# cchao0116/EasyDGL

Measured on AMD Instinct MI355X. Metric: sequences/sec (fwd+bwd+Adam) B=512 L=100 d=128 |I|=20K, higher is better.
Workload: dtype bf16

## Files before the change

### easydgl_amd/build.py

```python
from __future__ import annotations

import hashlib
import os
import subprocess
import sys
from concurrent.futures import ThreadPoolExecutor

HERE = os.path.dirname(os.path.abspath(__file__))
CSRC = os.path.join(HERE, "csrc")
OUT = os.path.join(HERE, "libeasydgl_hip.so")
SOURCES = ["k_misc.hip", "k_tpp.hip", "k_optim.hip", "k_adam_rows.hip", "k_reduce.hip", "k_data.hip", "k_encode.hip", "k_gemm.hip", "k_gemm2.hip", "k_layernorm.hip", "k_bimau_fwd.hip", "k_bimau_bwd.hip", "k_bimau_big.hip", "k_bimau_stream.hip",
           "k_score.hip", "k_ce.hip", "k_score_strip.hip", "k_score_stripw.hip", "k_eval_tile.hip", "k_eval_topk.hip", "k_eval_rank.hip", "k_eval_cand.hip", "k_cand_ce.hip", "k_shared_ce.hip", "k_sampled_loss.hip", "k_tattn.hip", "k_tiattn.hip", "k_timefn.hip", "k_coding.hip", "k_tail.hip", "k_segsum.hip", "k_gru.hip", "k_s2pnm.hip", "k_mate.hip", "k_tahe.hip"]
HEADERS = ["edgl_common.h", "lds_limit.h", "batch_prep.h", "tpp_math.h", "score_plan.h", "topk_select.h", "gemm_tile.h", "bimau_common.h", "bimau_fwd_impl.h", "bimau_bwd_impl.h", "red_batch.h", "tn_group.h", "encode_scatter.h", "strip_mma.h", "score_strip.h", "eval_sweep.h", "cand_gather.h", "sampled_dv.h", "tattn_common.h", os.path.join("..", "..", "include", "easydgl_hip.h")]
FLAGS = ["--offload-arch=gfx950", "-O3", "-std=c++17", "-fPIC", "-munsafe-fp-atomics", "-Wno-unused-result"]
EXTRA_FLAGS = {"k_bimau_fwd.hip": ["-mllvm", "-amdgpu-mfma-vgpr-form=1"],
               "k_bimau_bwd.hip": ["-mllvm", "-amdgpu-mfma-vgpr-form=1"],
               "k_bimau_big.hip": ["-mllvm", "-amdgpu-mfma-vgpr-form=1"],
               "k_bimau_stream.hip": ["-mllvm", "-amdgpu-mfma-vgpr-form=1"],
               "k_tattn.hip": ["-mllvm", "-amdgpu-mfma-vgpr-form=1"],
               "k_tiattn.hip": ["-mllvm", "-amdgpu-mfma-vgpr-form=1"],
               "k_timefn.hip": ["-mllvm", "-amdgpu-mfma-vgpr-form=1"],
               "k_score_strip.hip": ["-fno-slp-vectorize", "-Wno-unused-value"] + (["-DSTRIP_SAFE"] if os.environ.get("EDGL_STRIP_SAFE") else []),
               "k_score_stripw.hip": ["-fno-slp-vectorize", "-Wno-unused-value"] + (["-DSTRIP_SAFE"] if os.environ.get("EDGL_STRIP_SAFE") else [])}


def _hipcc() -> str:
    for c in (os.environ.get("HIPCC"), "/opt/rocm/bin/hipcc", "hipcc"):
        if c and (os.path.isabs(c) and os.path.exists(c) or not os.path.isabs(c)):
            return c
    raise RuntimeError("hipcc not found")


def _digest(paths, extra=()) -> str:
    h = hashlib.sha256()
    for e in extra:
        h.update(str(e).encode() + b"\0")
    for p in paths:
        with open(p, "rb") as f:
            h.update(os.path.basename(p).encode() + b"\0" + f.read() + b"\0")
    return h.hexdigest()


def _stamp_ok(target: str, digest: str) -> bool:
    stamp = target + ".sha256"
    return os.path.exists(target) and os.path.exists(stamp) and open(stamp).read().strip() == digest


def _write_stamp(target: str, digest: str) -> None:
    with open(target + ".sha256", "w") as f:
        f.write(digest + "\n")


def build(force: bool = False, verbose: bool = False) -> str:
    hipcc = _hipcc()
    objdir = os.path.join(CSRC, "obj")
    os.makedirs(objdir, exist_ok=True)
    hdrs = [os.path.join(CSRC, h) for h in HEADERS]
    jobs = []
    digests = {}
    for src in SOURCES:
        s = os.path.join(CSRC, src)
        o = os.path.join(objdir, src.replace(".hip", ".o"))
        digests[o] = _digest([s] + hdrs, FLAGS + EXTRA_FLAGS.get(src, []))
        if force or not _stamp_ok(o, digests[o]):
            jobs.append((s, o))

    def run(job):
        s, o = job
        cmd = [hipcc] + FLAGS + EXTRA_FLAGS.get(os.path.basename(s), []) + ["-c", s, "-o", o]
        r = subprocess.run(cmd, capture_output=True, text=True)
        if r.returncode != 0:
            raise RuntimeError("hipcc failed for %s:\n%s" % (s, r.stderr[-4000:]))
        _write_stamp(o, digests[o])
        if verbose:
            print("compiled", os.path.basename(s))
        return o

    if jobs:
        with ThreadPoolExecutor(max_workers=min(8, len(jobs))) as ex:
            list(ex.map(run, jobs))
    objs = [os.path.join(objdir, s.replace(".hip", ".o")) for s in SOURCES]
    link_digest = _digest([], [digests[o] for o in objs])
    if force or jobs or not _stamp_ok(OUT, link_digest):
        cmd = [hipcc, "--offload-arch=gfx950", "-shared", "-fPIC", "-o", OUT] + objs
        r = subprocess.run(cmd, capture_output=True, text=True)
        if r.returncode != 0:
            raise RuntimeError("link failed:\n" + r.stderr[-4000:])
        _write_stamp(OUT, link_digest)
    return OUT


if __name__ == "__main__":
    print(build(force="--force" in sys.argv, verbose=True))
```

### easydgl_amd/csrc/bimau_bwd_impl.h

```cpp
#pragma once
#include <algorithm>

#include "bimau_common.h"

#ifdef EDGL_PHASE_TIMING
extern __device__ unsigned long long g_phase_cycles[16];
#endif

namespace bimau {


constexpr int KY_ECH = 8;
constexpr int KY_NY = EP / KY_ECH;
constexpr int KY_BLOCKS = 384;

constexpr int WG_NJ64 = 4;
constexpr int big_nj(int dh) { return dh == 64 ? WG_NJ64 : 32 / (dh / 16); }
inline int big_row_splits(int dh, int E) {
    const int nc = big_nj(dh) * 16;
    const int groups = std::max(1, (dh * E + nc - 1) / nc);
    return std::max(16, 512 / groups);
}

struct WsLayout { size_t dz, dh, rowdot, dsc, wpart, total; };
inline WsLayout ws_layout(int B, int T_, int C, int H, int E, long dsc_rows = 0) {
    const int dh = C / H;
    const bool big = dh >= 64;
    const size_t R = (size_t)B * H * T_;
    WsLayout w;
    size_t o = 0;
    auto take = [&](size_t bytes) { const size_t at = o; o += (bytes + 255) & ~(size_t)255; return at; };
    w.dz = take(R * EP * sizeof(float));
    w.dh = take((size_t)(big ? 1 : KY_NY) * R * dh * sizeof(float));
    w.rowdot = take(R * sizeof(float));
    w.dsc = take((size_t)(dsc_rows > 0 ? dsc_rows : (long)B * H) * EP * sizeof(float));
    w.wpart = take((size_t)(big ? big_row_splits(dh, E) : KY_BLOCKS) * ((size_t)(dh + 3) * dh * E + EP) * sizeof(float));
    w.total = o;
    return w;
}

struct BwdP {
    const void* qkvt; const int64_t* ids; const float* spans; const uint8_t* marks; const char* pack;
    const void* d_out; const float* d_lam_ext; const float* lam; const float* z; const void* hin;
    int B, T, C, H, E;
    float rate; const uint64_t* rng; uint32_t stream_id;
    void* d_qkvt;
    float* dz_ws; float* dh_ws; float* rowdot_ws; float* dsc_part; float* wpart;
    int waves;
    int flags;
    int noskip;
    const uint32_t* dbits;
    float qk_scale;
    const void* tpp_desc; int tpp_M; const float* tpp_sums; float tpp_coef;
    const int32_t* order;
    float* tpp_part;
};

template <typename T>
__device__ __forceinline__ void st_frag(T* dst, const f32x4& a) {
    Frag4<T> f = frag_from_acc<T>(a);
    if constexpr (sizeof(T) == 4) *reinterpret_cast<uint4*>(dst) = *reinterpret_cast<uint4*>(&f);
    else *reinterpret_cast<uint2*>(dst) = *reinterpret_cast<uint2*>(&f);
}

template <typename T, int DT, int NT, int EC, bool PREF = true, int FL = -1, bool DB = false, bool TP = false, bool SK = false>
__global__ __launch_bounds__(256) void bimau_bwd_sweep1_kernel(BwdP p) {
    constexpr int dh = 16 * DT, Tp = 16 * NT, LDT = Tp + 4;
    extern __shared__ __attribute__((aligned(16))) char smem[];
    const int E = EC ? EC : p.E;
    const int lane = threadIdx.x & 63, wave = __builtin_amdgcn_readfirstlane(threadIdx.x >> 6);
    const long slot = (long)blockIdx.x * p.waves + wave;
    if (slot >= (long)p.B * p.H) return;
    const int sb = (int)(slot / p.H), head = (int)(slot % p.H);
    const int b = p.order ? __builtin_amdgcn_readfirstlane(p.order[sb]) : sb;
    const long job = (long)b * p.H + head;
    const long bp = (long)head * p.B + b;
    const int g4 = (lane >> 4) * 4, l15 = lane & 15;
    constexpr bool SWZ = img_swz<T>();
    const int g4s = SWZ ? swz_col<16>(l15, g4) : g4;
    int cw[DT];
#pragma unroll
    for (int ub = 0; ub < DT; ++ub) cw[ub] = SWZ ? swz_col<16 * DT>(l15, ub * 16 + g4) : ub * 16 + g4;

    constexpr bool TR = sizeof(T) == 2;
    constexpr size_t EXTRA = TR ? 0 : (size_t)EP * LDT;
    constexpr size_t MASK_ELEMS = (size_t)Tp * sizeof(float) / sizeof(T);
    constexpr size_t WAVE_ELEMS = 2 * (size_t)Tp * dh + (size_t)Tp * EP + EXTRA + MASK_ELEMS;
    T* Ks = reinterpret_cast<T*>(smem) + (size_t)wave * WAVE_ELEMS;
    T* Vs = Ks + Tp * dh;
    T* Ms = Vs + Tp * dh;
    T* MTs = Ms + Tp * EP;
    const T* qkvt = reinterpret_cast<const T*>(p.qkvt) + (long)b * p.T * 4 * p.C;
    const T* dout = reinterpret_cast<const T*>(p.d_out) + (long)b * p.T * p.C;
    T* dqkvt = reinterpret_cast<T*>(p.d_qkvt) + (long)b * p.T * 4 * p.C;
    const int ldq = 4 * p.C;
    const KeyMask<NT> km = stage_wave<T, DT, NT, EC>(
        qkvt + p.C + head * dh, Ks, nullptr, static_cast<const T*>(nullptr), static_cast<T*>(nullptr), static_cast<T*>(nullptr),
        qkvt + 2 * p.C + head * dh, Vs, nullptr, ldq, p.marks + (long)b * p.T * E, E, Ms, TR ? nullptr : MTs,
        p.ids + (long)b * p.T, reinterpret_cast<float*>(Ks + WAVE_ELEMS - MASK_ELEMS), p.T, LDT, lane);
    __builtin_amdgcn_fence(__ATOMIC_RELEASE, "wavefront");
    __builtin_amdgcn_wave_barrier();

    const PackDims pd = pack_dims<T>(dh, E);
    const float* iscs_g = reinterpret_cast<const float*>(p.pack + pd.off_f32) + 3 * pd.JE + EP;
    float isc[4];
#pragma unroll
    for (int i = 0; i < 4; ++i) isc[i] = iscs_g[g4 + i];

    const float cscale = p.qk_scale > 0.f ? p.qk_scale : rsqrtf((float)dh);
    const DropKey dk = make_dropkey(p.rng, p.stream_id, p.rate);
    const Frag4<T> ident = identity_frag<T>(lane);
    const f32x4 zero4 = {0.f, 0.f, 0.f, 0.f};

    struct QOps { Frag4<T> qf[DT], dof[DT]; float4 z; float lam[4], dlx[4]; uint32_t kb; uint32_t nmw; float spr; };
    const float* dlx_src = p.d_lam_ext ? p.d_lam_ext : p.lam;
    const float dlx_on = p.d_lam_ext ? 1.0f : 0.0f;
    TppDesc td{};
    int tp_novf = 0;
    float tp_k = 0.f;
    if constexpr (TP) {
        td = tpp_desc(p.tpp_desc, p.B, p.T, p.tpp_M);
        tp_novf = __builtin_amdgcn_readfirstlane(td.novf[b]);
        int cnt;
        if (p.tpp_sums) {
            cnt = reinterpret_cast<const int*>(p.tpp_sums)[4];
        } else {
            cnt = 0;
            for (int i = lane; i < p.B; i += 64) cnt += td.cntp[i];
            for (int o = 32; o > 0; o >>= 1) cnt += __shfl_xor(cnt, o, 64);
        }
        tp_k = -p.tpp_coef / ((float)cnt * (float)p.H);
        if (job == 0 && lane == 0) reinterpret_cast<int*>(p.tpp_part)[2 * p.B * p.H] = cnt;
    }
    auto load_q = [&](int qt) {
        QOps o;
        const int q = min(qt * 16 + l15, p.T - 1);
        const long row = bp * p.T + q;
#pragma unroll
        for (int ub = 0; ub < DT; ++ub) {
            o.qf[ub] = frag_ld<T>(qkvt + (long)q * ldq + head * dh + ub * 16 + g4);
            o.dof[ub] = frag_ld<T>(dout + (long)q * p.C + head * dh + ub * 16 + g4);
        }
        o.z = *reinterpret_cast<const float4*>(p.z + row * EP + g4);
        if constexpr (DB) o.kb = p.dbits[(bp * NT + qt) * 64 + lane];
        if constexpr (TP) {
            const float4 l4 = *reinterpret_cast<const float4*>(p.lam + row * EC + g4);
            o.lam[0] = l4.x; o.lam[1] = l4.y; o.lam[2] = l4.z; o.lam[3] = l4.w;
            o.dlx[0] = 0.f; o.dlx[1] = 0.f; o.dlx[2] = 0.f; o.dlx[3] = 0.f;
            o.nmw = td.nmw[((long)b * p.T + q) * 4 + (lane >> 4)];
            o.spr = td.spr[(long)b * p.T + q];
        } else if constexpr (EC == 16) {
            const float4 l4 = *reinterpret_cast<const float4*>(p.lam + row * EC + g4), d4 = *reinterpret_cast<const float4*>(dlx_src + row * EC + g4);
            o.lam[0] = l4.x; o.lam[1] = l4.y; o.lam[2] = l4.z; o.lam[3] = l4.w;
            o.dlx[0] = d4.x; o.dlx[1] = d4.y; o.dlx[2] = d4.z; o.dlx[3] = d4.w;
        } else {
#pragma unroll
            for (int i = 0; i < 4; ++i) {
                const int e = min(g4 + i, E - 1);
                o.lam[i] = p.lam[row * E + e];
                o.dlx[i] = dlx_src[row * E + e];
            }
        }
        return o;
    };
    auto mask_q = [&](QOps& o, bool ok) {
#pragma unroll
        for (int ub = 0; ub < DT; ++ub)
            if (!ok) o.dof[ub] = frag_zero<T>();
#pragma unroll
        for (int i = 0; i < 4; ++i) {
            const bool oke = ok && (EC == 16 || (g4 + i) < E);
            o.lam[i] = oke ? o.lam[i] : 0.f;
            o.dlx[i] = oke ? o.dlx[i] * dlx_on : 0.f;
        }
    };
    PH_DECL
    auto run = [&](auto nk_c) {
    constexpr int NK = decltype(nk_c)::value, K0 = NT - NK;
    const KeyMask<NK> kmk = keymask_tail<NK, NT>(km);
    float dsc_acc[4] = {0.f, 0.f, 0.f, 0.f}, tp_a = 0.f, tp_b = 0.f;
    f32x4 dVa[DT][NK];
#pragma unroll
    for (int u = 0; u < DT; ++u)
#pragma unroll
        for (int kt = 0; kt < NK; ++kt) dVa[u][kt] = zero4;
    QOps qcur = load_q(0);
    touch_regs(qcur);
    float pend_dz[4] = {0.f, 0.f, 0.f, 0.f}, pend_rowdot = 0.f;
    int pend_q = p.T;
    auto flush_pending = [&]() {
        if (pend_q < p.T) {
            *reinterpret_cast<float4*>(p.dz_ws + (bp * p.T + pend_q) * EP + g4) = make_float4(pend_dz[0], pend_dz[1], pend_dz[2], pend_dz[3]);
            if (lane < 16) p.rowdot_ws[bp * p.T + pend_q] = pend_rowdot;
        }
    };
    for (int qt = 0; qt < NT; ++qt) {
        asm volatile("" ::: "memory");
        const int q = qt * 16 + l15;
        const bool qok = q < p.T;
        QOps qnext;
        if constexpr (PREF) qnext = load_q(qt + 1 < NT ? qt + 1 : qt);
        asm volatile("" ::: "memory");
        mask_q(qcur, qok);
        if constexpr (TP) {
            float gr[4] = {0.f, 0.f, 0.f, 0.f};
            tpp_slot(qcur.lam, qcur.nmw, qcur.spr, qok && qcur.spr >= 0.f, tp_k, gr, tp_a, tp_b);
            for (int j = 0; j < tp_novf; ++j) {
                const int tj = td.ovf_pos[(long)b * td.M + j];
                if ((tj >> 4) != qt) continue;
                tpp_slot(qcur.lam, td.ovf_nm[((long)b * td.M + j) * 4 + (lane >> 4)], qcur.spr, qok && q == tj, tp_k, gr, tp_a, tp_b);
            }
#pragma unroll
            for (int i = 0; i < 4; ++i) qcur.dlx[i] = gr[i];
        }
        const float zq4[4] = {qcur.z.x, qcur.z.y, qcur.z.z, qcur.z.w};
        f32x4 s[NK];
#pragma unroll
        for (int kt = 0; kt < NK; ++kt) {
            f32x4 a = zero4;
#pragma unroll
            for (int ub = 0; ub < DT; ++ub)
                a = mma16(frag_ld<T>(Ks + ((K0 + kt) * 16 + l15) * dh + cw[ub]), qcur.qf[ub], a);
            s[kt] = a;
        }
// ... 415 lines not shown
```

### easydgl_amd/csrc/k_bimau_big.hip

```cpp
#include "bimau_bwd_impl.h"
#include "bimau_fwd_impl.h"
#include <type_traits>

namespace {
using namespace bimau;

struct IntP {
    const void* hin; const float* spans; const char* pack; const float* dz;
    long R; int B, T, E;
    float* z_out; float* lam;
    float* dh_out;
    float* wpart; const float* dsc_part; long njobs;
};

__device__ __forceinline__ void copy16(const char* src, char* dst, int bytes) {
    for (int i = threadIdx.x * 16; i < bytes; i += blockDim.x * 16)
        *reinterpret_cast<uint4*>(dst + i) = *reinterpret_cast<const uint4*>(src + i);
}

typedef unsigned int u32x4 __attribute__((ext_vector_type(4)));
typedef unsigned int u32x2 __attribute__((ext_vector_type(2)));
template <typename T, int DT, bool WITH_R>
struct MarkChunk {
    static constexpr int dh = 16 * DT, LDC = dh + 4;
// ... 306 lines not shown
        for (int r = 0; r < 4; ++r) {
            const int q = min(qt * 16 + g4 + r, p.T - 1);
            o.spn[r] = p.spans[(long)bb * p.T + q];
            o.dz0[r] = p.dz[(rowq + q) * EP + e_lo];
            o.dz1[r] = p.dz[(rowq + q) * EP + e_hi];
        }
        return o;
    };
    const long tstep = (long)gridDim.x * 4;
    long t = (long)blockIdx.x * 4 + wave;
    Pre cur = load_tile(t);
    for (; t < ntile; t += tstep) {
        const Pre nxt = load_tile(t + tstep);
        const long bpq = t / ntq; const int qt = (int)(t - bpq * ntq);
        const bool okA = qt * 16 + l15 < p.T;
        Frag4<T> hA[DT], hB[DT];
#pragma unroll
        for (int ub = 0; ub < DT; ++ub) {
            hA[ub] = okA ? cur.hA[ub] : frag_zero<T>();
            hB[ub] = frag_from_acc<T>(mma16(hA[ub], ident, zero4));
        }
        float spn[4];
        bool rok[4];
#pragma unroll
        for (int r = 0; r < 4; ++r) {
            rok[r] = qt * 16 + g4 + r < p.T;
            spn[r] = rok[r] ? cur.spn[r] : 0.f;
        }
#pragma unroll
        for (int jj = 0; jj < NJ; ++jj) {
            const bool hi_mark = (j0 + jj * 16) / dh > e_lo;
            f32x4 a = zero4;
#pragma unroll
            for (int ub = 0; ub < DT; ++ub) a = mma16(hA[ub], frag_ld<T>(Wc + (jj * 16 + l15) * LDW + ub * 16 + g4), a);
            const float ws = fc[jj * 16 + l15], bs = fc[NC + jj * 16 + l15], wv = fc[2 * NC + jj * 16 + l15];
            f32x4 du;
            float sdb = 0.f, sdws = 0.f, sdw = 0.f;
#pragma unroll
            for (int r = 0; r < 4; ++r) {
                const float dz = rok[r] ? (hi_mark ? cur.dz1[r] : cur.dz0[r]) : 0.f;
                const float z = sigmoid_pre(fmaf(spn[r], ws, a[r]) + bs);
                const float t2 = dz * z;
                du[r] = t2 * wv * (1.0f - z);
                sdb += du[r]; sdws += du[r] * spn[r]; sdw += t2;
            }
            adb[jj] += sdb; adws[jj] += sdws; adw[jj] += sdw;
            const Frag4<T> duf = frag_from_acc<T>(du);
#pragma unroll
            for (int ub = 0; ub < DT; ++ub) dW[jj][ub] = mma16(duf, hB[ub], dW[jj][ub]);
        }
        cur = nxt;
    }
    for (int w = 0; w < 4; ++w) {
        if (wave == w) {
#pragma unroll
            for (int jj = 0; jj < NJ; ++jj) {
                const float sb = group_sum4(adb[jj]), sws = group_sum4(adws[jj]), sw = group_sum4(adw[jj]);
                if (lane < 16) {
                    accs[dh * NC + jj * 16 + l15] += sws;
                    accs[(dh + 1) * NC + jj * 16 + l15] += sb;
                    accs[(dh + 2) * NC + jj * 16 + l15] += sw;
                }
#pragma unroll
                for (int ub = 0; ub < DT; ++ub)
#pragma unroll
                    for (int r = 0; r < 4; ++r) accs[(ub * 16 + l15) * NC + jj * 16 + g4 + r] += dW[jj][ub][r];
            }
        }
        __syncthreads();
    }
    float* dst = p.wpart + (long)blockIdx.x * NPARX;
    for (int i = threadIdx.x; i < (dh + 3) * NC; i += blockDim.x)
        if ((i % NC) < nval) dst[(long)(i / NC) * JE + j0 + (i % NC)] = accs[i];
    if (blockIdx.y == 0 && threadIdx.x < EP) {
        const long per = (p.njobs + gridDim.x - 1) / gridDim.x;
        const long a0 = blockIdx.x * per, a1 = min(p.njobs, a0 + per);
        float a = 0.f;
        for (long j = a0; j < a1; ++j) a += p.dsc_part[j * EP + threadIdx.x];
        dst[NPAR + threadIdx.x] = a;
    }
}

inline int row_blocks(long ntile, int tiles_per_wg) {
    return (int)std::max<long>(1, std::min<long>((ntile + tiles_per_wg - 1) / tiles_per_wg, 1024));
}

template <typename T, int DT>
int run_intensity_fwd(const FwdP& p, hipStream_t st) {
    constexpr int dh = 16 * DT;
    IntP ip{};
    ip.hin = p.hin_out; ip.spans = p.spans; ip.pack = p.pack; ip.R = (long)p.B * p.H * p.T; ip.B = p.B; ip.T = p.T; ip.E = p.E;
    ip.z_out = p.z_out; ip.lam = p.lam;
    const size_t smem = (size_t)MarkChunk<T, DT, false>::BYTES * (big_double_buffer<T, DT>() ? 2 : 1);
    auto k = intensity_fwd_big_kernel<T, DT>;
    EDGL_LDS_LIMIT(k, smem, "edgl_bimau_fwd");
    const long ntile = (long)p.B * p.H * ((p.T + 15) / 16);
    hipLaunchKernelGGL(k, dim3(row_blocks(ntile, 8)), dim3(256), smem, st, ip);
    EDGL_LAUNCH_CHECK();
    return EDGL_OK;
}

template <typename T, int DT, int NT>
int fwd_big(FwdP p, hipStream_t st) {
    int rc = launch_fwd_e<T, DT, NT, 0, 1>(p, st);
    if (rc) return rc;
    rc = run_intensity_fwd<T, DT>(p, st);
    if (rc) return rc;
    return launch_fwd_e<T, DT, NT, 0, 2>(p, st);
}

template <typename T, int DT>
int run_intensity_bwd_big(const BwdP& p, long dsc_rows, hipStream_t st) {
    constexpr int dh = 16 * DT;
    const long jobs = (long)p.B * p.H;
    const int JE = dh * p.E;
    const int RS = big_row_splits(dh, p.E);
    IntP ip{};
    ip.hin = p.hin; ip.spans = p.spans; ip.pack = p.pack; ip.dz = p.dz_ws; ip.R = (long)p.B * p.H * p.T; ip.B = p.B; ip.T = p.T;
    ip.E = p.E; ip.dh_out = p.dh_ws; ip.wpart = p.wpart; ip.dsc_part = p.dsc_part; ip.njobs = dsc_rows;
    const long ntile = jobs * ((p.T + 15) / 16);
    const size_t smem_r = (size_t)MarkChunk<T, DT, true>::BYTES * (big_double_buffer<T, DT>() ? 2 : 1);
    auto kr = intensity_bwd_rows_big_kernel<T, DT>;
    EDGL_LDS_LIMIT(kr, smem_r, "edgl_bimau_bwd");
    hipLaunchKernelGGL(kr, dim3(row_blocks(ntile, 8)), dim3(256), smem_r, st, ip);
    EDGL_LAUNCH_CHECK();
    constexpr int NC = WGroup<DT>::NJ * 16;
    const size_t smem_w = (size_t)NC * (dh + 4) * sizeof(T) + (size_t)(3 * NC + (dh + 3) * NC) * sizeof(float);
    auto kw = intensity_bwd_weights_big_kernel<T, DT>;
    EDGL_LDS_LIMIT(kw, smem_w, "edgl_bimau_bwd");
    hipLaunchKernelGGL(kw, dim3(RS, (JE + NC - 1) / NC), dim3(256), smem_w, st, ip);
    EDGL_LAUNCH_CHECK();
    return EDGL_OK;
}

template <typename T, int DT, int NT>
int bwd_big(BwdP p, char* ws, float* dW1, float* db1, float* dw, float* dscaling, hipStream_t st) {
    constexpr int dh = 16 * DT, Tp = 16 * NT, LDT = Tp + 4;
    constexpr bool TR = sizeof(T) == 2;
    const WsLayout wl = ws_layout(p.B, p.T, p.C, p.H, p.E);
    p.dz_ws = reinterpret_cast<float*>(ws + wl.dz); p.dh_ws = reinterpret_cast<float*>(ws + wl.dh);
    p.rowdot_ws = reinterpret_cast<float*>(ws + wl.rowdot);
    p.dsc_part = reinterpret_cast<float*>(ws + wl.dsc); p.wpart = reinterpret_cast<float*>(ws + wl.wpart);
    const long jobs = (long)p.B * p.H;
    edgl_prof_begin(EDGL_KERNEL_BIMAU_BWD_ALL, st);
    {
        const size_t wave_bytes = (2 * (size_t)Tp * dh + (size_t)Tp * EP + (TR ? 0 : (size_t)EP * LDT)) * sizeof(T) + (size_t)Tp * sizeof(float);
        int waves = 4;
        while (waves > 1 && waves * wave_bytes > 64 * 1024) waves >>= 1;
        const size_t smem = waves * wave_bytes;
        EDGL_REQUIRE(smem <= 160 * 1024, EDGL_ERR_SHAPE, "edgl_bimau_bwd: sweep 1 needs %zu B of LDS (dh=%d T=%d)", smem, dh, p.T);
        p.waves = waves;
        auto kern = bimau_bwd_sweep1_kernel<T, DT, NT, 0, false>;
        EDGL_LDS_LIMIT(kern, smem, "edgl_bimau_bwd");
        hipLaunchKernelGGL(kern, dim3((unsigned)((jobs + waves - 1) / waves)), dim3(64 * waves), smem, st, p);
        EDGL_LAUNCH_CHECK();
    }
    {
        const int rc = run_intensity_bwd_big<T, DT>(p, jobs, st);
        if (rc) return rc;
    }
    {
        const size_t wave_bytes = (3 * (size_t)Tp * dh + (size_t)Tp * EP + (TR ? 0 : (size_t)dh * LDT)) * sizeof(T) + (size_t)Tp * sizeof(float);
        int waves = 4;
        while (waves > 1 && waves * wave_bytes > 80 * 1024) waves >>= 1;
        const size_t smem = waves * wave_bytes;
        EDGL_REQUIRE(smem <= 160 * 1024, EDGL_ERR_SHAPE, "edgl_bimau_bwd: sweep 2 needs %zu B of LDS (dh=%d T=%d)", smem, dh, p.T);
        p.waves = waves;
        edgl_prof_begin(EDGL_KERNEL_BIMAU_BWD, st);
        if constexpr (DT * NT > 32) {
            auto k0 = bimau_bwd_sweep2_kernel<T, DT, NT, 0, 1, false, -1, false, 2, 0>;
            auto k1 = bimau_bwd_sweep2_kernel<T, DT, NT, 0, 1, false, -1, false, 2, 1>;
            EDGL_LDS_LIMIT(k0, smem, "edgl_bimau_bwd");
            EDGL_LDS_LIMIT(k1, smem, "edgl_bimau_bwd");
            hipLaunchKernelGGL(k0, dim3((unsigned)((jobs + waves - 1) / waves)), dim3(64 * waves), smem, st, p);
            hipLaunchKernelGGL(k1, dim3((unsigned)((jobs + waves - 1) / waves)), dim3(64 * waves), smem, st, p);
        } else {
            auto kern = bimau_bwd_sweep2_kernel<T, DT, NT, 0, 1, false>;
            EDGL_LDS_LIMIT(kern, smem, "edgl_bimau_bwd");
            hipLaunchKernelGGL(kern, dim3((unsigned)((jobs + waves - 1) / waves)), dim3(64 * waves), smem, st, p);
        }
        edgl_prof_end(EDGL_KERNEL_BIMAU_BWD, st);
        edgl_prof_end(EDGL_KERNEL_BIMAU_BWD_ALL, st);
        EDGL_LAUNCH_CHECK();
    }
    return reduce_wparts(p.wpart, big_row_splits(dh, p.E), dh, p.E, dW1, db1, dw, dscaling, st);
}

constexpr bool big_ok(size_t esize, int DT, int NT) { return esize == 2 ? NT <= 8 : (DT == 4 ? NT <= 7 : NT <= 4); }
template <typename T, int DT, int NT>
int fwd_big_or_error(const FwdP& p, hipStream_t st) {
    if constexpr (big_ok(sizeof(T), DT, NT)) return fwd_big<T, DT, NT>(p, st);
    edgl_set_error("edgl_bimau_fwd: head dim %d with T=%d in f32 not supported (f32: dh 64: T <= 112, dh 128: T <= 64; bf16: T <= 128)", 16 * DT, p.T);
    return EDGL_ERR_SHAPE;
}
template <typename T>
int fwd_dispatch(const FwdP& p, hipStream_t st) {
    const int dh = p.C / p.H, nt = (p.T + 15) / 16;
#define EDGL_BIG_CASES(DT_)                                                                                              \
    switch (nt) {                                                                                                        \
        case 1: return fwd_big_or_error<T, DT_, 1>(p, st); case 2: return fwd_big_or_error<T, DT_, 2>(p, st);            \
        case 3: return fwd_big_or_error<T, DT_, 3>(p, st); case 4: return fwd_big_or_error<T, DT_, 4>(p, st);            \
        case 5: return fwd_big_or_error<T, DT_, 5>(p, st); case 6: return fwd_big_or_error<T, DT_, 6>(p, st);            \
        case 7: return fwd_big_or_error<T, DT_, 7>(p, st); case 8: return fwd_big_or_error<T, DT_, 8>(p, st);            \
    }
    if (dh == 64) { EDGL_BIG_CASES(4) } else if (dh == 128) { EDGL_BIG_CASES(8) }
#undef EDGL_BIG_CASES
    edgl_set_error("edgl_bimau_fwd: head dim %d with T=%d not supported (head dims 64 / 128: T <= 128)", dh, p.T);
    return EDGL_ERR_SHAPE;
}
template <typename T, int DT, int NT>
int bwd_big_or_error(const BwdP& p, char* ws, float* dW1, float* db1, float* dw, float* dsc, hipStream_t st) {
    if constexpr (big_ok(sizeof(T), DT, NT)) return bwd_big<T, DT, NT>(p, ws, dW1, db1, dw, dsc, st);
    edgl_set_error("edgl_bimau_bwd: head dim %d with T=%d in f32 not supported (f32: dh 64: T <= 112, dh 128: T <= 64; bf16: T <= 128)", 16 * DT, p.T);
    return EDGL_ERR_SHAPE;
}
template <typename T>
int bwd_dispatch(const BwdP& p, char* ws, float* dW1, float* db1, float* dw, float* dsc, hipStream_t st) {
    const int dh = p.C / p.H, nt = (p.T + 15) / 16;
#define EDGL_BIG_CASES(DT_)                                                                                                            \
    switch (nt) {                                                                                                                      \
        case 1: return bwd_big_or_error<T, DT_, 1>(p, ws, dW1, db1, dw, dsc, st); case 2: return bwd_big_or_error<T, DT_, 2>(p, ws, dW1, db1, dw, dsc, st); \
        case 3: return bwd_big_or_error<T, DT_, 3>(p, ws, dW1, db1, dw, dsc, st); case 4: return bwd_big_or_error<T, DT_, 4>(p, ws, dW1, db1, dw, dsc, st); \
        case 5: return bwd_big_or_error<T, DT_, 5>(p, ws, dW1, db1, dw, dsc, st); case 6: return bwd_big_or_error<T, DT_, 6>(p, ws, dW1, db1, dw, dsc, st); \
        case 7: return bwd_big_or_error<T, DT_, 7>(p, ws, dW1, db1, dw, dsc, st); case 8: return bwd_big_or_error<T, DT_, 8>(p, ws, dW1, db1, dw, dsc, st); \
    }
    if (dh == 64) { EDGL_BIG_CASES(4) } else if (dh == 128) { EDGL_BIG_CASES(8) }
#undef EDGL_BIG_CASES
    edgl_set_error("edgl_bimau_bwd: head dim %d with T=%d not supported (head dims 64 / 128: T <= 128)", dh, p.T);
    return EDGL_ERR_SHAPE;
}

}

namespace bimau {
int big_fwd(const FwdP& p, int dtype, hipStream_t st) {
    if (!p.hin_out || !p.z_out) {
        edgl_set_error("edgl_bimau_fwd: head dims >= 64 run as three launches and need `saved` (edgl_bimau_saved_bytes) as scratch, also for inference");
        return EDGL_ERR_WORKSPACE;
    }
    return dtype == EDGL_F32 ? fwd_dispatch<float>(p, st) : fwd_dispatch<bf16>(p, st);
}
int big_bwd(const BwdP& p, char* ws, float* dW1, float* db1, float* dw, float* dsc, int dtype, hipStream_t st) {
    return dtype == EDGL_F32 ? bwd_dispatch<float>(p, ws, dW1, db1, dw, dsc, st) : bwd_dispatch<bf16>(p, ws, dW1, db1, dw, dsc, st);
}
int intensity_fwd_rows(const FwdP& p, int dtype, hipStream_t st) {
    const bool f = dtype == EDGL_F32;
    switch (p.C / p.H) {
        case 16: return f ? run_intensity_fwd<float, 1>(p, st) : run_intensity_fwd<bf16, 1>(p, st);
        case 32: return f ? run_intensity_fwd<float, 2>(p, st) : run_intensity_fwd<bf16, 2>(p, st);
        case 64: return f ? run_intensity_fwd<float, 4>(p, st) : run_intensity_fwd<bf16, 4>(p, st);
        case 128: return f ? run_intensity_fwd<float, 8>(p, st) : run_intensity_fwd<bf16, 8>(p, st);
    }
    edgl_set_error("edgl_bimau_fwd: head dim %d not supported (16, 32, 64 or 128)", p.C / p.H);
    return EDGL_ERR_SHAPE;
}
int intensity_bwd_big(const BwdP& p, long dsc_rows, float* dW1, float* db1, float* dw, float* dsc, int dtype, hipStream_t st) {
    const bool f = dtype == EDGL_F32;
    const int dh = p.C / p.H;
    int rc;
    if (dh == 64) rc = f ? run_intensity_bwd_big<float, 4>(p, dsc_rows, st) : run_intensity_bwd_big<bf16, 4>(p, dsc_rows, st);
    else if (dh == 128) rc = f ? run_intensity_bwd_big<float, 8>(p, dsc_rows, st) : run_intensity_bwd_big<bf16, 8>(p, dsc_rows, st);
    else { edgl_set_error("edgl_bimau_bwd: head dim %d has no streamed-weights intensity backward (64 or 128)", dh); return EDGL_ERR_SHAPE; }
    if (rc) return rc;
    return reduce_wparts(p.wpart, big_row_splits(dh, p.E), dh, p.E, dW1, db1, dw, dsc, st);
}
}
```

### easydgl_amd/csrc/k_bimau_bwd.hip

```cpp
#include <algorithm>
#include <cstdlib>

#include "bimau_bwd_impl.h"

#ifdef EDGL_PHASE_TIMING
__device__ unsigned long long g_phase_cycles[16];
#endif

namespace {
using namespace bimau;

template <typename T>
constexpr int intensity_bwd_nreg(int DT) {
    return KY_ECH * DT * DT * 4 + (sizeof(T) == 2 ? (KY_ECH / 4) * DT * 4 : 2 * KY_ECH * DT) + KY_ECH * DT;
}

struct MlpP {
    const void* hin; const float* dz_ws; const float* spans; const char* pack;
    long R; int B, T, E; float* dh_ws; float* wpart; const float* dsc_part; long njobs;
    int slab_epi;
};

template <typename T, int DT, int EC>
__global__ __launch_bounds__(256, (sizeof(T) == 2 && DT == 1) ? 3 : 1) void intensity_bwd_kernel(MlpP p) {
// ... 194 lines not shown
                    slab[(RX + (ee * DT + d) * 2 + 1) * 64] = adws[ee][d];
                }
                slab[(RW + ee * DT + d) * 64] = adw[ee][d];
            }
        __syncthreads();
        const float* sl = reinterpret_cast<const float*>(smem);
        auto sum4 = [&](int reg, int ln) {
            const float* q = sl + reg * 64 + ln;
            return (q[0] + q[NREG * 64]) + (q[2 * NREG * 64] + q[3 * NREG * 64]);
        };
        for (int i = threadIdx.x; i < NPAR; i += blockDim.x) {
            const int row = i / JE, j = i - row * JE;
            const int jt = j >> 4, jl = j & 15, e = jt / DT, d = jt - e * DT, ee = e - e0;
            if (ee < 0 || ee >= ECH) continue;
            float v;
            if (row < dh) {
                v = sum4((((ee * DT + d) * DT + (row >> 4)) * 4) + (jl & 3), (jl >> 2) * 16 + (row & 15));
            } else if (row == dh + 2) {
                const int reg = RW + ee * DT + d;
                v = (sum4(reg, jl) + sum4(reg, 16 + jl)) + (sum4(reg, 32 + jl) + sum4(reg, 48 + jl));
            } else if constexpr (MX) {
                const int reg = RX + ((ee / 4) * DT + d) * 4 + (jl & 3), ln = (jl >> 2) * 16 + 3 * (ee % 4);
                v = row == dh + 1 ? sum4(reg, ln) : sum4(reg, ln + 1) + sum4(reg, ln + 2);
            } else {
                const int reg = RX + (ee * DT + d) * 2 + (row == dh ? 1 : 0);
                v = (sum4(reg, jl) + sum4(reg, 16 + jl)) + (sum4(reg, 32 + jl) + sum4(reg, 48 + jl));
            }
            p.wpart[(long)blockIdx.x * NPARX + i] = v;
        }
    } else {
    for (int w = 0; w < 4; ++w) {
        if (wave == w) {
#pragma unroll
            for (int ee = 0; ee < ECH; ++ee) {
                const int e = e0 + ee;
                if (EC == 16 || e < E) {
#pragma unroll
                    for (int d = 0; d < DT; ++d) {
                        const int jt = e * DT + d;
                        const float sw = group_sum4(adw[ee][d]);
                        if (lane < 16) accs[WROW + 2 * JE + jt * 16 + l15] += sw;
                        if constexpr (MX) {
                            const int c0 = 3 * (ee % 4);
#pragma unroll
                            for (int r = 0; r < 4; ++r) {
                                const float x = dWx[ee / 4][d][r];
                                const float nb = __int_as_float(__builtin_amdgcn_update_dpp(0, __float_as_int(x), 0x101, 0xf, 0xf, true));
                                const int j = jt * 16 + g4 + r;
                                if (l15 == c0 || l15 == c0 + 1) accs[l15 == c0 ? WROW + JE + j : WROW + j] += l15 == c0 ? x : x + nb;
                            }
                        } else {
                            const float sb = group_sum4(adb[ee][d]), sws = group_sum4(adws[ee][d]);
                            if (lane < 16) {
                                const int j = jt * 16 + l15;
                                accs[WROW + j] += sws;
                                accs[WROW + JE + j] += sb;
                            }
                        }
#pragma unroll
                        for (int ub = 0; ub < DT; ++ub)
#pragma unroll
                            for (int r = 0; r < 4; ++r) {
                                const int j = jt * 16 + g4 + r, u = ub * 16 + l15;
                                accs[j * (dh + 1) + u] += dW[ee][d][ub][r];
                            }
                    }
                }
            }
        }
        __syncthreads();
    }
    for (int i = threadIdx.x; i < NPAR; i += blockDim.x) {
        const int e = (i % JE) / dh;
        const int row = i / JE, j = i - row * JE;
        if (e >= e0 && e < e0 + ECH) p.wpart[(long)blockIdx.x * NPARX + i] = row < dh ? accs[j * (dh + 1) + row] : accs[WROW + (row - dh) * JE + j];
    }
    }
    if (blockIdx.y == 0) {
        const long per = (p.njobs + gridDim.x - 1) / gridDim.x;
        const long j0 = blockIdx.x * per, j1 = min(p.njobs, j0 + per);
        const int e = threadIdx.x & 15, sl = threadIdx.x >> 4;
        float a = 0.f;
        for (long j = j0 + sl; j < j1; j += 16) a += p.dsc_part[j * EP + e];
        __syncthreads();
        accs[sl * EP + e] = a;
        __syncthreads();
        if (threadIdx.x < EP) {
            float v = 0.f;
#pragma unroll
            for (int k = 0; k < 16; ++k) v += accs[k * EP + threadIdx.x];
            p.wpart[(long)blockIdx.x * NPARX + NPAR + threadIdx.x] = v;
        }
    }
    PH_MARK(7);
    PH_FLUSH(0);
}

template <typename T>
size_t intensity_bwd_lds(int dh, int E) {
    const int NACC = dh * E * (dh + 4);
    return pack_dims<T>(dh, E).bytes + ((size_t)((NACC + 3) & ~3) + 4 * (16 * KY_ECH + 16)) * sizeof(float);
}

template <typename T, int DT>
int launch_intensity_bwd(const BwdP& p, long dsc_rows, hipStream_t st) {
    constexpr int dh = 16 * DT;
    MlpP mp{p.hin, p.dz_ws, p.spans, p.pack, (long)p.B * p.H * p.T, p.B, p.T, p.E, p.dh_ws, p.wpart, p.dsc_part, dsc_rows, 0};
    size_t smem_b = intensity_bwd_lds<T>(dh, p.E);
    const size_t slab_b = (size_t)4 * intensity_bwd_nreg<T>(DT) * 64 * sizeof(float);
    mp.slab_epi = slab_b <= std::max(smem_b, (size_t)52 * 1024);
    if (mp.slab_epi) smem_b = std::max(smem_b, slab_b);
    EDGL_REQUIRE(smem_b <= 160 * 1024, EDGL_ERR_SHAPE, "edgl_bimau_bwd: intensity kernel needs %zu B of LDS", smem_b);
    EDGL_REQUIRE((long)p.B * p.H * p.T < (1l << 31) - 16, EDGL_ERR_SHAPE, "edgl_bimau_bwd: B*H*T = %ld rows exceed the 32-bit row index", (long)p.B * p.H * p.T);
    auto kb = intensity_bwd_kernel<T, DT, 0>;
    EDGL_LDS_LIMIT(kb, smem_b, "edgl_bimau_bwd");
    hipLaunchKernelGGL(kb, dim3(KY_BLOCKS, KY_NY), dim3(256), smem_b, st, mp);
    EDGL_LAUNCH_CHECK();
    return EDGL_OK;
}

template <typename T, int DT, int NT>
int launch_bwd(BwdP p, char* ws, float* dW1, float* db1, float* dw, float* dscaling, hipStream_t st) {
    constexpr int dh = 16 * DT, Tp = 16 * NT, LDT = Tp + 4;
    const PackDims pd = pack_dims<T>(dh, p.E);
    const WsLayout wl = ws_layout(p.B, p.T, p.C, p.H, p.E);
    p.dz_ws = reinterpret_cast<float*>(ws + wl.dz); p.dh_ws = reinterpret_cast<float*>(ws + wl.dh);
    p.rowdot_ws = reinterpret_cast<float*>(ws + wl.rowdot);
    p.dsc_part = reinterpret_cast<float*>(ws + wl.dsc); p.wpart = reinterpret_cast<float*>(ws + wl.wpart);
    const long jobs = (long)p.B * p.H;
    constexpr bool TR = sizeof(T) == 2;
    edgl_prof_begin(EDGL_KERNEL_BIMAU_BWD_ALL, st);
    {
        const size_t wave_bytes = (2 * (size_t)Tp * dh + (size_t)Tp * EP + (TR ? 0 : (size_t)EP * LDT)) * sizeof(T) + (size_t)Tp * sizeof(float);
        int waves = 4;
        while (waves > 1 && waves * wave_bytes > 64 * 1024) waves >>= 1;
        const size_t smem = waves * wave_bytes;
        p.waves = waves;
        constexpr bool SPEC = sizeof(T) == 2 && DT == 1;
        auto kern = p.E == 16 ? bimau_bwd_sweep1_kernel<T, DT, NT, 16> : bimau_bwd_sweep1_kernel<T, DT, NT, 0>;
        if constexpr (SPEC) {
            if (p.flags == 0) kern = p.E == 16 ? bimau_bwd_sweep1_kernel<T, DT, NT, 16, true, 0> : bimau_bwd_sweep1_kernel<T, DT, NT, 0, true, 0>;
            if constexpr (NT <= 8) {
                constexpr bool SKC = NT >= 2;
                const bool sk = SKC && p.flags == 0 && p.E == 16 && bimau_skip_enabled() && !p.noskip;
                const bool db = p.dbits && p.rate > 0.f;
                if (p.flags == 0 && p.E == 16 && db) kern = sk ? bimau_bwd_sweep1_kernel<T, DT, NT, 16, true, 0, true, false, SKC> : bimau_bwd_sweep1_kernel<T, DT, NT, 16, true, 0, true>;
                else if (sk) kern = bimau_bwd_sweep1_kernel<T, DT, NT, 16, true, 0, false, false, SKC>;
                if (p.tpp_desc) {
                    if (sk) kern = db ? bimau_bwd_sweep1_kernel<T, DT, NT, 16, true, 0, true, true, SKC> : bimau_bwd_sweep1_kernel<T, DT, NT, 16, true, 0, false, true, SKC>;
                    else kern = db ? bimau_bwd_sweep1_kernel<T, DT, NT, 16, true, 0, true, true> : bimau_bwd_sweep1_kernel<T, DT, NT, 16, true, 0, false, true>;
                }
            }
        }
        EDGL_LDS_LIMIT(kern, smem, "edgl_bimau_bwd");
        hipLaunchKernelGGL(kern, dim3((unsigned)((jobs + waves - 1) / waves)), dim3(64 * waves), smem, st, p);
        EDGL_LAUNCH_CHECK();
    }
    {
        const int rc = launch_intensity_bwd<T, DT>(p, jobs, st);
        if (rc) return rc;
    }
    {
        const size_t wave_bytes = (3 * (size_t)Tp * dh + (size_t)Tp * EP + (TR ? 0 : (size_t)dh * LDT)) * sizeof(T) + (size_t)Tp * sizeof(float);
        int waves = 4;
        while (waves > 1 && waves * wave_bytes > 80 * 1024) waves >>= 1;
        const size_t smem = waves * wave_bytes;
        EDGL_REQUIRE(smem <= 160 * 1024, EDGL_ERR_SHAPE, "edgl_bimau_bwd: needs %zu B of LDS", smem);
        p.waves = waves;
        constexpr bool SPEC = sizeof(T) == 2 && DT == 1;
        auto kern = p.E == 16 ? bimau_bwd_sweep2_kernel<T, DT, NT, 16> : bimau_bwd_sweep2_kernel<T, DT, NT, 0>;
        if constexpr (SPEC) {
            if (p.flags == 0) kern = p.E == 16 ? bimau_bwd_sweep2_kernel<T, DT, NT, 16, KY_NY, true, 0> : bimau_bwd_sweep2_kernel<T, DT, NT, 0, KY_NY, true, 0>;
            if constexpr (NT <= 8) {
                constexpr bool SKC = NT >= 2;
                const bool sk = SKC && p.flags == 0 && p.E == 16 && bimau_skip_enabled() && !p.noskip;
                if (p.flags == 0 && p.E == 16 && p.dbits && p.rate > 0.f) kern = sk ? bimau_bwd_sweep2_kernel<T, DT, NT, 16, KY_NY, true, 0, true, 1, 0, SKC> : bimau_bwd_sweep2_kernel<T, DT, NT, 16, KY_NY, true, 0, true>;
                else if (sk) kern = bimau_bwd_sweep2_kernel<T, DT, NT, 16, KY_NY, true, 0, false, 1, 0, SKC>;
            }
        }
        EDGL_LDS_LIMIT(kern, smem, "edgl_bimau_bwd");
        edgl_prof_begin(EDGL_KERNEL_BIMAU_BWD, st);
        hipLaunchKernelGGL(kern, dim3((unsigned)((jobs + waves - 1) / waves)), dim3(64 * waves), smem, st, p);
        edgl_prof_end(EDGL_KERNEL_BIMAU_BWD, st);
        edgl_prof_end(EDGL_KERNEL_BIMAU_BWD_ALL, st);
        EDGL_LAUNCH_CHECK();
    }
    return reduce_wparts(p.wpart, KY_BLOCKS, dh, p.E, dW1, db1, dw, dscaling, st);
}

template <typename T, int DT>
int dispatch_nt(BwdP p, char* ws, float* dW1, float* db1, float* dw, float* dsc, hipStream_t st) {
    switch ((p.T + 15) / 16) {
        case 1: return launch_bwd<T, DT, 1>(p, ws, dW1, db1, dw, dsc, st);
        case 2: return launch_bwd<T, DT, 2>(p, ws, dW1, db1, dw, dsc, st);
        case 3: return launch_bwd<T, DT, 3>(p, ws, dW1, db1, dw, dsc, st);
        case 4: return launch_bwd<T, DT, 4>(p, ws, dW1, db1, dw, dsc, st);
        case 5: return launch_bwd<T, DT, 5>(p, ws, dW1, db1, dw, dsc, st);
        case 6: return launch_bwd<T, DT, 6>(p, ws, dW1, db1, dw, dsc, st);
        case 7: return launch_bwd<T, DT, 7>(p, ws, dW1, db1, dw, dsc, st);
        case 8: return launch_bwd<T, DT, 8>(p, ws, dW1, db1, dw, dsc, st);
        case 9: return launch_bwd<T, DT, 9>(p, ws, dW1, db1, dw, dsc, st);
        case 10: return launch_bwd<T, DT, 10>(p, ws, dW1, db1, dw, dsc, st);
        case 11: return launch_bwd<T, DT, 11>(p, ws, dW1, db1, dw, dsc, st);
        case 12: return launch_bwd<T, DT, 12>(p, ws, dW1, db1, dw, dsc, st);
        case 13: return launch_bwd<T, DT, 13>(p, ws, dW1, db1, dw, dsc, st);
    }
    edgl_set_error("edgl_bimau_bwd: T=%d not supported (T <= 208)", p.T);
    return EDGL_ERR_SHAPE;
}

}

namespace bimau {
int intensity_bwd_small(const BwdP& p, long dsc_rows, float* dW1, float* db1, float* dw, float* dsc, int dtype, hipStream_t st) {
    const bool f = dtype == EDGL_F32;
    const int dh = p.C / p.H;
    int rc;
    if (dh == 16) rc = f ? launch_intensity_bwd<float, 1>(p, dsc_rows, st) : launch_intensity_bwd<bf16, 1>(p, dsc_rows, st);
    else if (dh == 32) rc = f ? launch_intensity_bwd<float, 2>(p, dsc_rows, st) : launch_intensity_bwd<bf16, 2>(p, dsc_rows, st);
    else { edgl_set_error("edgl_bimau_bwd: head dim %d has no weights-in-LDS intensity backward (16 or 32)", dh); return EDGL_ERR_SHAPE; }
    if (rc) return rc;
    return reduce_wparts(p.wpart, KY_BLOCKS, dh, p.E, dW1, db1, dw, dsc, st);
}
}

extern "C" long edgl_bimau_bwd_workspace_ex(int B, int T, int C, int H, int E, int dtype, int flags) {
    if (H <= 0 || C % H) return -1;
    const int form = bimau::bimau_form(T, C, H, dtype == EDGL_BF16 ? EDGL_BF16 : EDGL_F32, flags);
    return (long)ws_layout_form(B, T, C, H, E, form).total;
}
extern "C" long edgl_bimau_bwd_workspace(int B, int T, int C, int H, int E, int dtype) {
    return edgl_bimau_bwd_workspace_ex(B, T, C, H, E, dtype, 0);
}

extern "C" int edgl_bimau_mark_group(int C, int H, int dtype) {
    if (H <= 0 || C % H || (dtype != EDGL_F32 && dtype != EDGL_BF16)) return -1;
    const int dh = C / H;
    if (dh >= 64) return bimau::EP;
    for (int E = bimau::EP; E >= 1; --E) {
        const size_t b = dtype == EDGL_BF16 ? intensity_bwd_lds<bf16>(dh, E) : intensity_bwd_lds<float>(dh, E);
        if (b <= 160 * 1024) return E;
    }
    return -1;
}

extern "C" int edgl_bimau_bwd_db(const void* qkvt, const int64_t* ids, const float* spans, const uint8_t* marks,
                                 const void* pack, const void* d_out, const float* d_lam_ext, const float* lam,
                                 const void* saved, int B, int T, int C, int H, int E, float drop_rate,
                                 const uint64_t* rng_state, uint32_t stream_id, const uint32_t* dropbits, float qk_scale, void* d_qkvt,
                                 float* dW1, float* db1, float* dw, float* dscaling, void* workspace, int flags, int dtype, void* stream);
extern "C" int edgl_bimau_bwd(const void* qkvt, const int64_t* ids, const float* spans, const uint8_t* marks,
                              const void* pack, const void* d_out, const float* d_lam_ext, const float* lam,
                              const void* saved, int B, int T, int C, int H, int E, float drop_rate,
                              const uint64_t* rng_state, uint32_t stream_id, void* d_qkvt, float* dW1, float* db1,
                              float* dw, float* dscaling, void* workspace, int flags, int dtype, void* stream) {
    return edgl_bimau_bwd_db(qkvt, ids, spans, marks, pack, d_out, d_lam_ext, lam, saved, B, T, C, H, E, drop_rate, rng_state, stream_id,
                             nullptr, 0.f, d_qkvt, dW1, db1, dw, dscaling, workspace, flags, dtype, stream);
}
static int bimau_bwd_impl(const void* qkvt, const int64_t* ids, const float* spans, const uint8_t* marks,
                          const void* pack, const void* d_out, const float* d_lam_ext, const float* lam,
                          const void* saved, int B, int T, int C, int H, int E, float drop_rate,
                          const uint64_t* rng_state, uint32_t stream_id, const uint32_t* dropbits, float qk_scale, void* d_qkvt,
                          float* dW1, float* db1, float* dw, float* dscaling, void* workspace, const void* tpp_desc, int tpp_M,
                          const float* tpp_sums, float tpp_coef, float* tpp_part, const int32_t* order, int flags, int dtype, void* stream) {
    EDGL_REQUIRE(qkvt && ids && spans && marks && pack && d_out && lam && saved && d_qkvt && dW1 && db1 && dw && dscaling && workspace,
                 EDGL_ERR_NULL, "edgl_bimau_bwd: null pointer");
    EDGL_REQUIRE(B > 0 && T > 0 && H > 0 && C % H == 0 && E >= 1 && E <= bimau::EP, EDGL_ERR_SHAPE,
                 "edgl_bimau_bwd: bad shape B=%d T=%d C=%d H=%d E=%d", B, T, C, H, E);
    EDGL_REQUIRE(dtype == EDGL_F32 || dtype == EDGL_BF16, EDGL_ERR_DTYPE, "edgl_bimau_bwd: bad dtype %d", dtype);
    EDGL_REQUIRE(drop_rate == 0.f || rng_state, EDGL_ERR_NULL, "edgl_bimau_bwd: dropout without rng_state");
    EDGL_REQUIRE((double)B * H * T * T < 4294967296.0, EDGL_ERR_SHAPE, "edgl_bimau_bwd: H*B*T*T must be < 2^32");
    BwdP p{};
    p.qkvt = qkvt; p.ids = ids; p.spans = spans; p.marks = marks; p.pack = (const char*)pack; p.d_out = d_out;
    p.d_lam_ext = d_lam_ext; p.lam = lam;
    const bimau::SavedLayout sl = bimau::saved_layout(B, T, C, H, dtype == EDGL_BF16 ? 2 : 4);
    p.hin = (const char*)saved + sl.off_hin;
    p.z = reinterpret_cast<const float*>((const char*)saved + sl.off_z);
    p.B = B; p.T = T; p.C = C; p.H = H; p.E = E; p.rate = drop_rate; p.rng = rng_state;
    p.noskip = (flags & EDGL_MAU_NO_SKIP) ? 1 : 0; flags &= ~EDGL_MAU_NO_SKIP;
    p.stream_id = stream_id; p.d_qkvt = d_qkvt; p.flags = flags; p.dbits = dropbits; p.qk_scale = qk_scale;
    p.tpp_desc = tpp_desc; p.tpp_M = tpp_M; p.tpp_sums = tpp_sums; p.tpp_coef = tpp_coef; p.tpp_part = tpp_part; p.order = order;
    EDGL_REQUIRE(!tpp_desc || (dtype == EDGL_BF16 && C / H == 16 && E == 16 && T <= 128 && flags == 0 && tpp_part && tpp_M > 0 && !d_lam_ext),
                 EDGL_ERR_SHAPE, "edgl_bimau_bwd_tpp: the fused TPP form exists for bf16, head dim 16, 16 marks, T <= 128, BiMAU flags "
                 "(C/H=%d E=%d T=%d flags=%d)", C / H, E, T, flags);
    hipStream_t st = (hipStream_t)stream;
    const int dh = C / H;
    char* ws = (char*)workspace;
    const int form = bimau::bimau_form(T, C, H, dtype, flags);
    p.flags = flags & ~EDGL_MAU_STREAM;
    if (form < 0) {
        edgl_set_error("edgl_bimau_bwd: head dim %d with T=%d not supported (head dims 16, 32, 64 or 128; T <= %d)", dh, T, bimau::STREAM_MAX_T);
        return EDGL_ERR_SHAPE;
    }
    if (form == 1) {
        EDGL_REQUIRE(!tpp_desc, EDGL_ERR_SHAPE, "edgl_bimau_bwd_tpp: the fused TPP form does not exist on the key-streamed path (T=%d, T <= 128)", T);
        const WsLayout wl = ws_layout_form(B, T, C, H, E, 1);
        p.dz_ws = reinterpret_cast<float*>(ws + wl.dz); p.dh_ws = reinterpret_cast<float*>(ws + wl.dh);
        p.rowdot_ws = reinterpret_cast<float*>(ws + wl.rowdot);
        p.dsc_part = reinterpret_cast<float*>(ws + wl.dsc); p.wpart = reinterpret_cast<float*>(ws + wl.wpart);
        const bimau::SavedLayoutStream ss = bimau::saved_layout_stream(B, T, C, H, dtype == EDGL_BF16 ? 2 : 4);
        return bimau::stream_bwd(p, reinterpret_cast<const float*>((const char*)saved + ss.off_stats), dW1, db1, dw, dscaling, dtype, st);
    }
    if (dtype == EDGL_F32) {
        if (dh == 16) return dispatch_nt<float, 1>(p, ws, dW1, db1, dw, dscaling, st);
        if (dh == 32) return dispatch_nt<float, 2>(p, ws, dW1, db1, dw, dscaling, st);
    } else {
        if (dh == 16) return dispatch_nt<bf16, 1>(p, ws, dW1, db1, dw, dscaling, st);
        if (dh == 32) return dispatch_nt<bf16, 2>(p, ws, dW1, db1, dw, dscaling, st);
    }
// ... 45 lines not shown
```

### easydgl_amd/csrc/k_gemm2.hip

```cpp
#include <cstdlib>

#include "edgl_common.h"
#include <cstring>
#include "encode_scatter.h"
#include "tn_group.h"

typedef __attribute__((ext_vector_type(4))) short tr_s16x4;

namespace gemm2 {

__device__ __forceinline__ uint2 tr_read(const bf16* tile, int ld, int k0, int z0, int lane) {
    const int G = lane >> 4, s = lane & 15;
    const bf16* p = tile + (k0 + 4 * G + (s >> 2)) * ld + z0 + 4 * (s & 3);
    tr_s16x4 v = __builtin_amdgcn_ds_read_tr16_b64_v4i16((__attribute__((address_space(3))) tr_s16x4*)p);
    return *reinterpret_cast<uint2*>(&v);
}
__device__ __forceinline__ bf16x8 tr_frag32(const bf16* tile, int ld, int k0, int z0, int lane) {
    bf16x8 f;
    *reinterpret_cast<uint2*>(&f) = tr_read(tile, ld, k0, z0, lane);
    *(reinterpret_cast<uint2*>(&f) + 1) = tr_read(tile, ld, k0 + 16, z0, lane);
    return f;
}

struct EpiP {
    const float* bias; void* aux; int flags;
};

__device__ __forceinline__ int xcd_virtual_id(int b, int grid, int n_real) {
    if (grid & 7) return b < n_real ? b : -1;
    const int v = (b & 7) * (grid >> 3) + (b >> 3);
    return v < n_real ? v : -1;
}
static inline int xcd_grid(int n_real) { return (n_real + 7) / 8 * 8; }
__device__ __forceinline__ void epi_store4(const EpiP& e, bf16* C, void* Cany, long idx, int n, float x[4]) {
    if (e.flags & EDGL_EPI_BIAS) {
        const float4 b = *reinterpret_cast<const float4*>(e.bias + n);
        x[0] += b.x; x[1] += b.y; x[2] += b.z; x[3] += b.w;
    }
    if (e.flags & EDGL_EPI_SAVE_PRE) {
        Frag4<bf16> f = frag_from_acc<bf16>(f32x4{x[0], x[1], x[2], x[3]});
        *reinterpret_cast<uint2*>(reinterpret_cast<bf16*>(e.aux) + idx) = *reinterpret_cast<uint2*>(&f);
    }
    if (e.flags & EDGL_EPI_GELU) {
#pragma unroll
        for (int r = 0; r < 4; ++r) x[r] = gelu_t<bf16>(x[r]);
    }
    if (e.flags & EDGL_EPI_RELU) {
#pragma unroll
        for (int r = 0; r < 4; ++r) x[r] = fmaxf(x[r], 0.f);
    }
    if (e.flags & EDGL_EPI_MUL_DGELU) {
        const Frag4<bf16> a = frag_ld<bf16>(reinterpret_cast<const bf16*>(e.aux) + idx);
#pragma unroll
        for (int r = 0; r < 4; ++r) x[r] *= dgelu_t<bf16>(to_f32(a.v[r]));
    }
    if (e.flags & EDGL_EPI_OUT_F32) {
        float* c = reinterpret_cast<float*>(Cany) + idx;
        if (e.flags & EDGL_EPI_ACCUM) {
            const float4 o = *reinterpret_cast<const float4*>(c);
            x[0] += o.x; x[1] += o.y; x[2] += o.z; x[3] += o.w;
        }
        *reinterpret_cast<float4*>(c) = make_float4(x[0], x[1], x[2], x[3]);
    } else {
        if (e.flags & EDGL_EPI_ACCUM) {
            const Frag4<bf16> o = frag_ld<bf16>(C + idx);
#pragma unroll
            for (int r = 0; r < 4; ++r) x[r] += to_f32(o.v[r]);
        }
        Frag4<bf16> f = frag_from_acc<bf16>(f32x4{x[0], x[1], x[2], x[3]});
        *reinterpret_cast<uint2*>(C + idx) = *reinterpret_cast<uint2*>(&f);
    }
}

constexpr int S_NT = 256;
constexpr int S_ZB = 64;

struct StripP {
    const bf16* A; const bf16* B; void* C;
    int M, N, K, lda, ldb, ldc;
    EpiP epi;
};

struct StripEpi {
    bf16* Ostage; float* OstageF; const float* bias64;
    bool staged, fstage;
    uint4 pre_aux[2][2], pre_c[2][2];
};
__device__ __forceinline__ void strip_prefetch_combine(const StripP& p, StripEpi& e, int m0, int n0, int lane) {
    if (e.fstage) {
#pragma unroll
        for (int ix = 0; ix < 2; ++ix)
#pragma unroll
            for (int q = 0; q < 2; ++q) {
                const int m = min(m0 + ix * 16 + q * 8 + (lane >> 3), p.M - 1);
                const long idx = (long)m * p.ldc + n0 + (lane & 7) * 8;
                if (p.epi.flags & EDGL_EPI_MUL_DGELU) e.pre_aux[ix][q] = *reinterpret_cast<const uint4*>(reinterpret_cast<const bf16*>(p.epi.aux) + idx);
                if (p.epi.flags & EDGL_EPI_ACCUM) e.pre_c[ix][q] = *reinterpret_cast<const uint4*>(reinterpret_cast<const bf16*>(p.C) + idx);
            }
    }
}
__device__ __forceinline__ void strip_epilogue(const StripP& p, StripEpi& e, f32x4 (&acc)[4][2], int m0, int n0, int lane) {
    constexpr int LDO = 64 + 8, LDOF = 64 + 4;
    const int g4 = (lane >> 4) * 4, l15 = lane & 15;
    bf16* const Ostage = e.Ostage;
    float* const OstageF = e.OstageF;
    if (e.staged) {
#pragma unroll
        for (int ix = 0; ix < 2; ++ix) {
#pragma unroll
            for (int jz = 0; jz < 4; ++jz) {
                const int n = n0 + jz * 16 + g4;
                float x[4] = {acc[jz][ix][0], acc[jz][ix][1], acc[jz][ix][2], acc[jz][ix][3]};
                {
                    const float4 bb = *reinterpret_cast<const float4*>(e.bias64 + jz * 16 + g4);
                    x[0] += bb.x; x[1] += bb.y; x[2] += bb.z; x[3] += bb.w;
                }
                if (p.epi.flags & EDGL_EPI_SAVE_PRE) {
                    const int m = m0 + ix * 16 + l15;
                    if (m < p.M) {
                        Frag4<bf16> f = frag_from_acc<bf16>(f32x4{x[0], x[1], x[2], x[3]});
                        *reinterpret_cast<uint2*>(reinterpret_cast<bf16*>(p.epi.aux) + (long)m * p.ldc + n) = *reinterpret_cast<uint2*>(&f);
                    }
                }
                if (p.epi.flags & EDGL_EPI_GELU) {
#pragma unroll
                    for (int r = 0; r < 4; ++r) x[r] = gelu_t<bf16>(x[r]);
                }
                if (p.epi.flags & EDGL_EPI_RELU) {
#pragma unroll
                    for (int r = 0; r < 4; ++r) x[r] = fmaxf(x[r], 0.f);
                }
                Frag4<bf16> f = frag_from_acc<bf16>(f32x4{x[0], x[1], x[2], x[3]});
                *reinterpret_cast<uint2*>(Ostage + l15 * LDO + jz * 16 + g4) = *reinterpret_cast<uint2*>(&f);
            }
            __builtin_amdgcn_fence(__ATOMIC_RELEASE, "wavefront");
            __builtin_amdgcn_wave_barrier();
#pragma unroll
            for (int q = 0; q < 2; ++q) {
                const int lrow = q * 8 + (lane >> 3), cv = lane & 7, m = m0 + ix * 16 + lrow;
                const uint4 d = *reinterpret_cast<const uint4*>(Ostage + lrow * LDO + cv * 8);
                if (m < p.M) *reinterpret_cast<uint4*>(reinterpret_cast<bf16*>(p.C) + (long)m * p.ldc + n0 + cv * 8) = d;
            }
            __builtin_amdgcn_wave_barrier();
        }
    } else if (e.fstage) {
#pragma unroll
        for (int ix = 0; ix < 2; ++ix) {
#pragma unroll
            for (int jz = 0; jz < 4; ++jz) {
                const float4 bb = *reinterpret_cast<const float4*>(e.bias64 + jz * 16 + g4);
                *reinterpret_cast<float4*>(OstageF + l15 * LDOF + jz * 16 + g4) =
                    make_float4(acc[jz][ix][0] + bb.x, acc[jz][ix][1] + bb.y, acc[jz][ix][2] + bb.z, acc[jz][ix][3] + bb.w);
            }
            __builtin_amdgcn_fence(__ATOMIC_RELEASE, "wavefront");
            __builtin_amdgcn_wave_barrier();
#pragma unroll
            for (int q = 0; q < 2; ++q) {
                const int lrow = q * 8 + (lane >> 3), cv = lane & 7, m = m0 + ix * 16 + lrow;
                const float4 lo = *reinterpret_cast<const float4*>(OstageF + lrow * LDOF + cv * 8);
                const float4 hi = *reinterpret_cast<const float4*>(OstageF + lrow * LDOF + cv * 8 + 4);
                float x[8] = {lo.x, lo.y, lo.z, lo.w, hi.x, hi.y, hi.z, hi.w};
                if (p.epi.flags & EDGL_EPI_MUL_DGELU) {
                    const bf16x8 a = *reinterpret_cast<const bf16x8*>(&e.pre_aux[ix][q]);
#pragma unroll
                    for (int r = 0; r < 8; ++r) x[r] *= dgelu_t<bf16>(to_f32(a[r]));
                }
                if (p.epi.flags & EDGL_EPI_ACCUM) {
                    const bf16x8 o = *reinterpret_cast<const bf16x8*>(&e.pre_c[ix][q]);
#pragma unroll
                    for (int r = 0; r < 8; ++r) x[r] += to_f32(o[r]);
                }
                const Frag4<bf16> f0 = frag_from_acc<bf16>(f32x4{x[0], x[1], x[2], x[3]});
                const Frag4<bf16> f1 = frag_from_acc<bf16>(f32x4{x[4], x[5], x[6], x[7]});
                uint4 d;
                *reinterpret_cast<uint2*>(&d) = *reinterpret_cast<const uint2*>(&f0);
                *(reinterpret_cast<uint2*>(&d) + 1) = *reinterpret_cast<const uint2*>(&f1);
                if (m < p.M) *reinterpret_cast<uint4*>(reinterpret_cast<bf16*>(p.C) + (long)m * p.ldc + n0 + cv * 8) = d;
            }
            __builtin_amdgcn_wave_barrier();
        }
    } else {
#pragma unroll
        for (int ix = 0; ix < 2; ++ix) {
            const int m = m0 + ix * 16 + l15;
            if (m < p.M) {
#pragma unroll
// ... 294 lines not shown
        for (int i = 0; i < 4; ++i) {
            const int m = m0 + wm * 64 + i * 16 + l15;
#pragma unroll
            for (int j = 0; j < 4; ++j) {
                const int n = n0 + wn * 64 + j * 16 + g4;
                float x[4] = {acc[i][j][0], acc[i][j][1], acc[i][j][2], acc[i][j][3]};
                if (m < p.M) epi_store4(p.epi, reinterpret_cast<bf16*>(p.C), p.C, (long)m * p.ldc + n, n, x);
            }
        }
        return;
    }
    bf16* Os = reinterpret_cast<bf16*>(smem);
#pragma unroll
    for (int j = 0; j < 4; ++j) {
        const int nl = wn * 64 + j * 16 + g4;
        float4 b4 = make_float4(0.f, 0.f, 0.f, 0.f);
        if (p.epi.flags & EDGL_EPI_BIAS) b4 = *reinterpret_cast<const float4*>(p.epi.bias + n0 + nl);
#pragma unroll
        for (int i = 0; i < 4; ++i) {
            const int ml = wm * 64 + i * 16 + l15;
            const Frag4<bf16> f = frag_from_acc<bf16>(f32x4{acc[i][j][0] + b4.x, acc[i][j][1] + b4.y, acc[i][j][2] + b4.z, acc[i][j][3] + b4.w});
            *reinterpret_cast<uint2*>(Os + ml * G_LDO + nl) = *reinterpret_cast<const uint2*>(&f);
        }
    }
    lds_barrier();
    if constexpr (MAP) {
        dx_encode_epilogue(*x, Os, mb0, mt, vid % nbn, n0, p.ldc);
        return;
    }
    bf16* C = reinterpret_cast<bf16*>(p.C);
#pragma unroll
    for (int i = 0; i < 8; ++i) {
        const int v = tid + i * G_NT, r = v >> 4, cpc = (v & 15) * 8;
        if (m0 + r < p.M) *reinterpret_cast<uint4*>(C + (long)(m0 + r) * p.ldc + n0 + cpc) = *reinterpret_cast<const uint4*>(Os + r * G_LDO + cpc);
    }
#undef G_AROW
#undef G_LOAD_ONE
#undef G_LOAD
#undef G_STORE_ONE
#undef G_STORE
}

template <bool B_KC, bool EPI = false>
__global__ __launch_bounds__(G_NT, EPI ? 2 : 3) void tile_nn_kernel(StripP p) {
    extern __shared__ __attribute__((aligned(16))) char smem[];
    const int vid = xcd_virtual_id((int)blockIdx.x, (int)gridDim.x, ((p.M + G_BM - 1) / G_BM) * (p.N / G_BN));
    if (vid < 0) return;
    tile_nn_tile<B_KC, EPI, false>(p, vid, smem, nullptr);
}

constexpr int DXE_LDS = G_BM * G_LDO * (int)sizeof(bf16) + 4 * enc_scatter::SROWS * 4;
__device__ __forceinline__ void dx_encode_epilogue(const DxEncP& x, bf16* Os, int mb0, int mt, int jn, int n0, int ldc) {
    using namespace enc_scatter;
    static_assert(G_LDO == 128 + 8 && G_BM == SROWS, "the output tile is the scatter's row image");
    constexpr int C = 128;
    const EncBwdP& e = x.e;
    int* s_id = reinterpret_cast<int*>(Os + G_BM * G_LDO);
    int* s_lead = s_id + SROWS;
    float* s_nm = reinterpret_cast<float*>(s_lead + SROWS);
    const int tid = threadIdx.x, T = x.mapT, B = x.mapB;
    if (x.dx0_out) {
#pragma unroll
        for (int i = 0; i < 8; ++i) {
            const int v = tid + i * G_NT, r = v >> 4, cpc = (v & 15) * 8;
            if (mb0 + r < B) *reinterpret_cast<uint4*>(x.dx0_out + ((long)(mb0 + r) * T + mt) * ldc + n0 + cpc) = *reinterpret_cast<const uint4*>(Os + r * G_LDO + cpc);
        }
        lds_barrier();
    }
    const int rl = tid >> 5, c0 = (tid & 31) * 4;
    const DropKey dk = make_dropkey(e.rng, e.stream_id, e.rate);
    if (jn == 0) {
        if (tid < SROWS) s_id[tid] = mb0 + tid < B ? (int)e.ids[(long)(mb0 + tid) * T + mt] : 0;
        const bool adds = e.add1 != nullptr;
        Frag4<bf16> ga[16], gb[16];
        if (adds) {
#pragma unroll
            for (int k = 0; k < 16; ++k) {
                const long row = (long)min(mb0 + rl + 8 * k, B - 1) * T + mt;
                ga[k] = frag_ld<bf16>(reinterpret_cast<const bf16*>(e.add1) + row * C + c0);
                gb[k] = frag_ld<bf16>(reinterpret_cast<const bf16*>(e.add2) + row * C + c0);
            }
        }
        lds_barrier();
        if (tid < SROWS) {
            const int lead = scatter_leader(s_id, tid);
            s_lead[tid] = s_id[tid] == 0 ? -1 : lead;
        }
#pragma unroll
        for (int k = 0; k < 16; ++k) {
            const int r = rl + 8 * k;
            const long row = (long)(mb0 + r) * T + mt;
            Frag4<bf16> v;
            *reinterpret_cast<uint2*>(&v) = *reinterpret_cast<const uint2*>(Os + r * G_LDO + c0);
            if (adds) {
#pragma unroll
                for (int j = 0; j < 4; ++j) v.v[j] = from_f32<bf16>(to_f32(v.v[j]) + to_f32(ga[k].v[j]) + to_f32(gb[k].v[j]));
            }
            if (dk.thresh != 0u) {
                const uint32_t keep = drop_keep4(dk, (uint64_t)row * 3 * C + c0);
#pragma unroll
                for (int j = 0; j < 4; ++j)
                    if (!((keep >> j) & 1u)) v.v[j] = from_f32<bf16>(0.f);
            }
            *reinterpret_cast<uint2*>(Os + r * G_LDO + c0) = *reinterpret_cast<const uint2*>(&v);
        }
        lds_barrier();
        scatter_onehot_sum<8>(Os, s_id, s_lead, e.d_item, C, 0, e.sq * dk.scale);
        return;
    }
    if (jn == 2) {
        if (mb0 == 0 && mt == 0 && e.d_mark_zero)
            for (int i = tid; i < e.E * C; i += G_NT) e.d_mark_zero[i] = 0.f;
        if (tid < SROWS) {
            int nm = 0;
            if (mb0 + tid < B) {
                const uint8_t* mrow = e.marks + ((long)(mb0 + tid) * T + mt) * e.E;
                for (int q = 0; q < e.E; ++q) nm += mrow[q];
            }
            s_nm[tid] = (float)nm;
        }
        lds_barrier();
    }
    double a[4] = {0., 0., 0., 0.};
#pragma unroll
    for (int k = 0; k < 16; ++k) {
        const int r = rl + 8 * k;
        if (mb0 + r < B) {
            const long row = (long)(mb0 + r) * T + mt;
            Frag4<bf16> g;
            *reinterpret_cast<uint2*>(&g) = *reinterpret_cast<const uint2*>(Os + r * G_LDO + c0);
            float v[4];
#pragma unroll
            for (int j = 0; j < 4; ++j) v[j] = to_f32(g.v[j]);
            drop_apply4(dk, (uint64_t)row * 3 * C + jn * C + c0, v);
            const double w = jn == 2 ? (double)s_nm[r] : 1.;
#pragma unroll
            for (int j = 0; j < 4; ++j) a[j] += w * (double)v[j];
        }
    }
    lds_barrier();
    double* sm = reinterpret_cast<double*>(Os);
    *reinterpret_cast<double2*>(sm + rl * C + c0) = make_double2(a[0], a[1]);
    *reinterpret_cast<double2*>(sm + rl * C + c0 + 2) = make_double2(a[2], a[3]);
    lds_barrier();
    if (tid < C) {
        double s = 0.;
#pragma unroll
        for (int i = 0; i < 8; ++i) s += sm[i * C + tid];
        float* part = jn == 1 ? e.part_pos : e.part_mk;
        part[((long)(mb0 / G_BM) * T + mt) * C + tid] = (float)s;
    }
}

template <int TM>
__device__ __forceinline__ void tn_body(const TnP& p, int bx, int by, int bz, bf16* Xs, bf16* Ys);

__global__ __launch_bounds__(G_NT, 3) void dx_encode_kernel(StripP p, DxEncP x, RedBatch rb, TnGroupP g, int tn_blocks) {
    static_assert(sizeof(StripP) + sizeof(DxEncP) + sizeof(RedBatch) + sizeof(TnGroupP) + sizeof(int) < 4096, "kernel arguments: 4 KB");
    static_assert(T_NT == G_NT && 2 * T_BR * T_LD * (int)sizeof(bf16) <= DXE_LDS, "the TN tiles run in this kernel's workgroup shape and LDS");
    extern __shared__ __attribute__((aligned(16))) char smem[];
    const int bid0 = (int)blockIdx.x;
    const int bid = bid0 - tn_blocks;
    if (bid0 < tn_blocks) {
        const int vid = xcd_virtual_id(bid0, tn_blocks, g.blk0[g.n]);
        if (vid < 0) return;
        int j = 0;
        for (int i = 1; i < g.n; ++i)
            if (vid >= g.blk0[i]) j = i;
        const int local = vid - g.blk0[j];
        const int tn = g.tiles_n[j], tk = g.tiles_k[j];
        bf16* Xs = reinterpret_cast<bf16*>(smem);
        tn_body<128>(g.job[j], local % tn, (local / tn) % tk, local / (tn * tk), Xs, Xs + T_BR * T_LD);
        return;
    }
    if (bid >= x.gemm_blocks) {
        const int e = bid - x.gemm_blocks;
        bf16* Gs = reinterpret_cast<bf16*>(smem);
        int* s_id = reinterpret_cast<int*>(Gs + G_BM * G_LDO);
        if (e < x.lab_blocks)
            enc_scatter::scatter_block<8>(x.e, x.e.lab_blk0 + e, 0, Gs, s_id, s_id + 128, reinterpret_cast<float*>(s_id + 256), reinterpret_cast<float*>(s_id + 384));
        else
            reduce_rows_vec_block(rb, e - x.lab_blocks, reinterpret_cast<float4(*)[9]>(smem));
        return;
    }
    const int vid = xcd_virtual_id(bid, x.gemm_blocks, (x.mapB + G_BM - 1) / G_BM * x.mapT * (p.N / G_BN));
    if (vid < 0) return;
    tile_nn_tile<true, false, true>(p, vid, smem, &x);
}

template <bool B_KC, bool EPI = false>
static int launch_tile_nn(const StripP& p, hipStream_t st) {
    constexpr size_t a_el = (size_t)G_BM * G_LDK, b_el = B_KC ? (size_t)G_BN * G_LDK : (size_t)G_BK * G_LDN;
    const size_t smem = std::max((EPI ? 2 : 1) * (a_el + b_el) * sizeof(bf16), (size_t)G_BM * G_LDO * sizeof(bf16));
    auto k = tile_nn_kernel<B_KC, EPI>;
    EDGL_LDS_LIMIT(k, smem, "edgl_gemm (tile)");
    const int nbm = (p.M + G_BM - 1) / G_BM, nbn = p.N / G_BN;
    hipLaunchKernelGGL(k, dim3((unsigned)xcd_grid(nbm * nbn)), dim3(G_NT), smem, st, p);
    EDGL_LAUNCH_CHECK();
    return 1;
}

template <int TM>
__device__ __forceinline__ void tn_body(const TnP& p, int bx, int by, int bz, bf16* Xs, bf16* Ys) {
    constexpr int NI = TM / 32, LDT = TM + 16, PCS = TM / 8, NLD = T_BR * PCS / T_NT;
    const int tid = threadIdx.x, lane = tid & 63, wave = tid >> 6, wm = wave >> 1, wn = wave & 1;
    const int g4 = (lane >> 4) * 4, l15 = lane & 15;
    const int kf0 = by * TM, n0 = bx * TM;
    const int r_lo = bz * p.rows_per_split, r_hi = min(p.R, r_lo + p.rows_per_split);
    f32x4 acc[NI][NI];
#pragma unroll
    for (int i = 0; i < NI; ++i)
#pragma unroll
        for (int j = 0; j < NI; ++j) acc[i][j] = f32x4{0.f, 0.f, 0.f, 0.f};
    constexpr int NCS = NI / 2;
    f32x4 acc_cs[NCS];
#pragma unroll
    for (int j = 0; j < NCS; ++j) acc_cs[j] = f32x4{0.f, 0.f, 0.f, 0.f};
    const bool do_cs = p.with_colsum && by == 0;
    bf16x8 ones;
#pragma unroll
    for (int i = 0; i < 8; ++i) ones[i] = (__bf16)1.0f;
    uint4 px[NLD], py[NLD];
    int r0_cur = 0;
    auto load = [&](int r0) {
        r0_cur = r0;
#pragma unroll
        for (int i = 0; i < NLD; ++i) {
            const int v = tid + i * T_NT, row = v / PCS, cv = v % PCS, gr = min(r0 + row, r_hi - 1);
            const int cx = min(kf0 + cv * 8, p.Kf - 8), cy = min(n0 + cv * 8, p.N - 8);
            px[i] = *reinterpret_cast<const uint4*>(p.X + (long)gr * p.ldx + cx);
            py[i] = *reinterpret_cast<const uint4*>(p.Y + (long)gr * p.ldy + cy);
        }
    };
    auto store = [&]() {
#pragma unroll
        for (int i = 0; i < NLD; ++i) {
            const int v = tid + i * T_NT, row = v / PCS, cv = v % PCS;
            const bool ok = r0_cur + row < r_hi;
            *reinterpret_cast<uint4*>(Xs + row * LDT + cv * 8) = ok ? px[i] : make_uint4(0, 0, 0, 0);
            *reinterpret_cast<uint4*>(Ys + row * LDT + cv * 8) = ok ? py[i] : make_uint4(0, 0, 0, 0);
        }
    };
    const int nstep = (r_hi - r_lo + T_BR - 1) / T_BR;
    if (nstep > 0) { load(r_lo); store(); }
    __syncthreads();
    for (int st = 0; st < nstep; ++st) {
        const bool more = st + 1 < nstep;
        if (more) load(r_lo + (st + 1) * T_BR);
#pragma unroll
        for (int rb = 0; rb < T_BR / 32; ++rb) {
            bf16x8 af[NI], bf_[NI];
#pragma unroll
            for (int i = 0; i < NI; ++i) af[i] = tr_frag32(Xs, LDT, rb * 32, wm * (TM / 2) + i * 16, lane);
#pragma unroll
            for (int j = 0; j < NI; ++j) bf_[j] = tr_frag32(Ys, LDT, rb * 32, wn * (TM / 2) + j * 16, lane);
#pragma unroll
            for (int i = 0; i < NI; ++i)
#pragma unroll
                for (int j = 0; j < NI; ++j) acc[i][j] = __builtin_amdgcn_mfma_f32_16x16x32_bf16(af[i], bf_[j], acc[i][j], 0, 0, 0);
            if (do_cs) {
                if (wm) {
#pragma unroll
                    for (int j = 0; j < NCS; ++j) acc_cs[j] = __builtin_amdgcn_mfma_f32_16x16x32_bf16(ones, bf_[NCS + j], acc_cs[j], 0, 0, 0);
                } else {
#pragma unroll
                    for (int j = 0; j < NCS; ++j) acc_cs[j] = __builtin_amdgcn_mfma_f32_16x16x32_bf16(ones, bf_[j], acc_cs[j], 0, 0, 0);
                }
            }
        }
        lds_barrier();
        if (more) store();
        lds_barrier();
    }
    float* out = p.partial + (long)bz * (p.Kf + 1) * p.N;
#pragma unroll
    for (int i = 0; i < NI; ++i)
#pragma unroll
        for (int r = 0; r < 4; ++r) {
            const int kf = kf0 + wm * (TM / 2) + i * 16 + g4 + r;
            if (kf < p.Kf) {
#pragma unroll
                for (int j = 0; j < NI; ++j) {
                    const int n = n0 + wn * (TM / 2) + j * 16 + l15;
                    if (n < p.N) out[(long)kf * p.N + n] = acc[i][j][r];
                }
            }
        }
    if (do_cs && lane < 16) {
#pragma unroll
        for (int j = 0; j < NCS; ++j) {
            const int n = n0 + wn * (TM / 2) + (wm * NCS + j) * 16 + lane;
            if (n < p.N) out[(long)p.Kf * p.N + n] = acc_cs[j][0];
        }
    }
}

template <int TM>
__global__ __launch_bounds__(T_NT) void tn_gemm_kernel(TnP p) {
    extern __shared__ __attribute__((aligned(16))) char tn_smem[];
    bf16* Xs = reinterpret_cast<bf16*>(tn_smem);
    bf16* Ys = Xs + T_BR * (TM + 16);
    const int vid = xcd_virtual_id((int)blockIdx.x, (int)gridDim.x, p.nblocks);
    if (vid < 0) return;
    tn_body<TM>(p, vid % p.tiles_n, (vid / p.tiles_n) % p.tiles_k, vid / (p.tiles_n * p.tiles_k), Xs, Ys);
}

__global__ __launch_bounds__(T_NT) void tn_gemm_group_kernel(TnGroupP g) {
    extern __shared__ __attribute__((aligned(16))) char tn_smem[];
    bf16* Xs = reinterpret_cast<bf16*>(tn_smem);
    bf16* Ys = Xs + T_BR * (128 + 16);
    const int vid = xcd_virtual_id((int)blockIdx.x, (int)gridDim.x, g.blk0[g.n]);
    if (vid < 0) return;
    int j = 0;
    for (int i = 1; i < g.n; ++i)
        if (vid >= g.blk0[i]) j = i;
    const int local = vid - g.blk0[j];
    const int tn = g.tiles_n[j], tk = g.tiles_k[j];
    tn_body<128>(g.job[j], local % tn, (local / tn) % tk, local / (tn * tk), Xs, Ys);
}

}

using namespace gemm2;

template <int NKB, bool B_KC>
static int launch_stream(const StripP& p, hipStream_t st) {
    constexpr int K = 32 * NKB;
    constexpr size_t cel = B_KC ? (size_t)64 * (K + 16) : (size_t)K * (64 + 16);
    const bool fstage = (p.epi.flags & (EDGL_EPI_ACCUM | EDGL_EPI_MUL_DGELU)) && !(p.epi.flags & EDGL_EPI_OUT_F32);
    const size_t smem = 2 * cel * sizeof(bf16) + (size_t)((p.N + 3) / 4 * 4) * sizeof(float) +
                        (fstage ? (size_t)8 * 16 * (64 + 4) * sizeof(float) : (size_t)8 * 16 * (64 + 8) * sizeof(bf16));
    if (smem > 160 * 1024) return 0;
    auto k = strip_stream_kernel<NKB, B_KC>;
    EDGL_LDS_LIMIT(k, smem, "edgl_gemm (stream)");
    hipLaunchKernelGGL(k, dim3((p.M + 255) / 256), dim3(W_NT), smem, st, p);
    EDGL_LAUNCH_CHECK();
    return 1;
}

template <int NKB, bool B_KC>
static int launch_strip(const StripP& p, hipStream_t st) {
    constexpr int K = 32 * NKB;
    constexpr size_t wel = B_KC ? (size_t)128 * (K + 16) : (size_t)K * (128 + 16);
    const bool fstage = (p.epi.flags & (EDGL_EPI_ACCUM | EDGL_EPI_MUL_DGELU)) && !(p.epi.flags & EDGL_EPI_OUT_F32);
    const size_t smem = wel * sizeof(bf16) + 128 * sizeof(float) +
                        (fstage ? (size_t)8 * 16 * (64 + 4) * sizeof(float) : (size_t)8 * 16 * (64 + 8) * sizeof(bf16));
    if (smem > 160 * 1024) return 0;
    auto k = strip_gemm_kernel<NKB, B_KC>;
    EDGL_LDS_LIMIT(k, smem, "edgl_gemm (strip)");
    const int nparts = (p.N + 127) / 128;
    const int per_cu = std::max(1, (int)((160 * 1024) / smem));
    const int nstrip8 = (p.M + 255) / 256;
    const int gx = std::max(1, std::min(nstrip8, (256 * std::min(per_cu, 2)) / nparts));
    hipLaunchKernelGGL(k, dim3(gx, nparts), dim3(W_NT), smem, st, p);
    EDGL_LAUNCH_CHECK();
    return 1;
}

int edgl_gemm2_try_strip(const void* A, const void* B, void* C, int M, int N, int K, int lda, int ldb, int ldc, int b_kc,
                         const float* bias, void* aux, int flags, hipStream_t st) {
    const bool ok = (K % 32 == 0) && K >= 32 && (N % 64 == 0) && (lda % 8 == 0) && (ldb % 8 == 0) &&
                    (ldc % 4 == 0) && (((uintptr_t)A | (uintptr_t)B | (uintptr_t)C) & 15) == 0 &&
                    (!aux || ((uintptr_t)aux & 7) == 0) && (!bias || ((uintptr_t)bias & 15) == 0);
    if (!ok) return 0;
    StripP p{(const bf16*)A, (const bf16*)B, C, M, N, K, lda, ldb, ldc, EpiP{bias, aux, flags}};
    int rc;
    if (M >= 4096 && N >= 256 && (N % G_BN) == 0 && (K % G_BK) == 0 && K >= 128 && (flags & ~EDGL_EPI_BIAS) == 0 &&
        (ldc % 8) == 0)
        return b_kc ? launch_tile_nn<true>(p, st) : launch_tile_nn<false>(p, st);
    if (K > 512) {
        if (M >= 1024 && (N % G_BN) == 0 && (K % G_BK) == 0)
            return b_kc ? launch_tile_nn<true, true>(p, st) : launch_tile_nn<false, true>(p, st);
        return 0;
    }
    if (N >= 384 && (K == 384 || K == 512) && M >= 4096) {
        rc = 0;
        if (K == 384) rc = b_kc ? launch_stream<12, true>(p, st) : launch_stream<12, false>(p, st);
        else rc = b_kc ? launch_stream<16, true>(p, st) : launch_stream<16, false>(p, st);
        if (rc) return rc;
    }
#define STRIP_CASE(NKB)                                                             \
    case NKB: rc = b_kc ? launch_strip<NKB, true>(p, st) : launch_strip<NKB, false>(p, st); break;
    switch (K / 32) {
        STRIP_CASE(1) STRIP_CASE(2) STRIP_CASE(4) STRIP_CASE(8) STRIP_CASE(12) STRIP_CASE(16)
        default: rc = 0;
    }
#undef STRIP_CASE
    if (rc == 0 && M >= 1024 && (N % G_BN) == 0 && (K % G_BK) == 0 && K >= 128)
        return b_kc ? launch_tile_nn<true, true>(p, st) : launch_tile_nn<false, true>(p, st);
    return rc;
}

static int tn_cus() {
    static const int cus = [] {
        int dev = 0, n = 0;
        if (hipGetDevice(&dev) != hipSuccess || hipDeviceGetAttribute(&n, hipDeviceAttributeMultiprocessorCount, dev) != hipSuccess || n <= 0) n = 256;
        return n;
    }();
    return cus;
}
static int tn_choose_splits(int R, int tiles, double flop, double out_elems, int cap) { return tn_choose_splits_on(tn_cus(), R, tiles, flop, out_elems, cap); }
static int tn_splits(int R, int Kf, int N) {
    const int tiles = ((Kf + 127) / 128) * ((N + 127) / 128);
    return tn_choose_splits(R, tiles, 2.0 * R * Kf * N, (double)(Kf + 1) * N, 1 << 20);
}
long edgl_gemm2_tn_workspace(int R, int Kf, int N) { return (long)tn_splits(R, Kf, N) * (Kf + 1) * N; }

static int tn_reduce(const float* workspace, int splits, float* C, int Kf, int N, float* dbias, int accumulate, hipStream_t st) {
    if (dbias && dbias == C + (long)Kf * N)
        return edgl_reduce_rows(workspace, splits, (Kf + 1) * N, (long)(Kf + 1) * N, C, accumulate, st);
    int rc = edgl_reduce_rows(workspace, splits, Kf * N, (long)(Kf + 1) * N, C, accumulate, st);
    if (rc) return rc;
    if (dbias) rc = edgl_reduce_rows(workspace + (long)Kf * N, splits, N, (long)(Kf + 1) * N, dbias, accumulate, st);
    return rc;
}

thread_local bool g_tn_defer = false;
thread_local int g_tn_n = 0;
thread_local TnQueued g_tn_q[TN_MAX_JOBS];
thread_local bool g_tn_ride = false;

static int tn_flush(hipStream_t st) {
    const int n = g_tn_n;
    g_tn_n = 0;
    if (n == 0) return EDGL_OK;
    TnGroupP g;
    int splits[TN_MAX_JOBS];
    const int blocks = tn_group_layout(g_tn_q, n, tn_cus(), &g, splits);
    const size_t tn_lds = (size_t)2 * T_BR * (128 + 16) * sizeof(bf16);
    EDGL_LDS_LIMIT(tn_gemm_group_kernel, tn_lds, "edgl_gemm_dw (grouped)");
    hipLaunchKernelGGL(tn_gemm_group_kernel, dim3(xcd_grid(blocks)), dim3(T_NT), tn_lds, st, g);
    EDGL_LAUNCH_CHECK();
    for (int i = 0; i < n; ++i) {
        const TnP& p = g_tn_q[i].p;
        const int rc = tn_reduce(p.partial, splits[i], g_tn_q[i].C, p.Kf, p.N, g_tn_q[i].dbias, g_tn_q[i].accumulate, st);
        if (rc) return rc;
    }
    return EDGL_OK;
}

int edgl_gemm2_tn_defer(int on, hipStream_t st) {
    if (on <= 0) g_tn_ride = false;
    if (on < 0) { g_tn_n = 0; g_tn_defer = false; return EDGL_OK; }
    if (!on && g_tn_defer) {
        g_tn_defer = false;
        return tn_flush(st);
    }
    g_tn_defer = on != 0;
    return EDGL_OK;
}

int edgl_gemm2_try_tn(const void* X, const void* Y, float* C, int R, int Kf, int N, int ldx, int ldy, int ldc, float* dbias,
                      int accumulate, float* workspace, hipStream_t st) {
    const bool ok = (Kf % 8 == 0) && (N % 8 == 0) && (ldx % 8 == 0) && (ldy % 8 == 0) && ldc == N &&
                    (((uintptr_t)X | (uintptr_t)Y) & 15) == 0 && workspace;
    if (!ok) return 0;
    int splits = tn_splits(R, Kf, N);
    int rps = ((R + splits - 1) / splits + T_BR - 1) / T_BR * T_BR;
    splits = (R + rps - 1) / rps;
    TnP p{(const bf16*)X, (const bf16*)Y, R, Kf, N, ldx, ldy, rps, workspace, dbias ? 1 : 0, 0, 0, 0};
    if (g_tn_defer) {
        if (g_tn_n == TN_MAX_JOBS) {
            const int rc = tn_flush(st);
            if (rc) return rc;
        }
        g_tn_q[g_tn_n++] = TnQueued{p, C, dbias, accumulate, splits};
        return 1;
    }
    const size_t lds = (size_t)2 * T_BR * (128 + 16) * sizeof(bf16);
    EDGL_LDS_LIMIT(tn_gemm_kernel<128>, lds, "edgl_gemm_dw");
    p.tiles_n = (N + 127) / 128; p.tiles_k = (Kf + 127) / 128; p.nblocks = p.tiles_n * p.tiles_k * splits;
    hipLaunchKernelGGL(tn_gemm_kernel<128>, dim3(xcd_grid(p.nblocks)), dim3(T_NT), lds, st, p);
    EDGL_LAUNCH_CHECK();
    const int rc = tn_reduce(workspace, splits, C, Kf, N, dbias, accumulate, st);
    return rc ? rc : 1;
}

extern "C" int edgl_gemm_dw_ride(int on) {
    EDGL_REQUIRE(on == 0 || on == 1, EDGL_ERR_SHAPE, "edgl_gemm_dw_ride: on = %d (0: off, 1: the queued products ride in the launch of edgl_dx_encode_bwd_label)", on);
    g_tn_ride = on != 0;
    return EDGL_OK;
}

extern "C" int edgl_dx_encode_supported(int B, int T, int C, int dtype) {
    if (dtype != EDGL_BF16 || C != 128 || B <= 0 || T <= 0) return 0;
    const int chunks = (B + G_BM - 1) / G_BM;
    return chunks <= enc_scatter::ENC_NCHUNK && (long)(chunks * G_BM - B) * 8 <= B ? 1 : 0;
}

extern "C" int edgl_dx_encode_bwd_label(const void* dqkvt, const void* W, int lda, int ldb, void* dx0_out, const int64_t* ids,
                                        const uint8_t* marks, const void* add1, const void* add2, int B, int T, int C, int E, int I,
                                        float drop_rate, const uint64_t* rng_state, uint32_t stream_id, float* d_item, float* d_pos,
                                        float* d_mark_emb, float* workspace, int c_true, const void* lab_rows, const int64_t* lab_ids,
                                        const float* lab_coef, const int32_t* lab_nvalid, int lab_R, float* d_bias, int dtype, void* stream) {
    using namespace enc_scatter;
    EDGL_REQUIRE(dqkvt && W && ids && marks && d_item && d_pos && d_mark_emb && workspace, EDGL_ERR_NULL, "edgl_dx_encode_bwd_label: null pointer");
    EDGL_REQUIRE(lab_rows && lab_ids && lab_coef && d_bias && lab_R > 0, EDGL_ERR_NULL, "edgl_dx_encode_bwd_label: null label operands");
    EDGL_REQUIRE((add1 == nullptr) == (add2 == nullptr), EDGL_ERR_NULL, "edgl_dx_encode_bwd_label: add1 / add2 go together");
    EDGL_REQUIRE(dtype == EDGL_BF16, EDGL_ERR_DTYPE, "edgl_dx_encode_bwd_label: bf16 only (dtype %d): f32 takes edgl_gemm + edgl_encode_bwd_add_ct", dtype);
    EDGL_REQUIRE(B > 0 && T > 0 && E >= 1 && I > 1 && edgl_dx_encode_supported(B, T, C, dtype), EDGL_ERR_SHAPE,
                 "edgl_dx_encode_bwd_label: needs bf16, C = 128, <= 16 chunks of 128 samples with at most B / 8 padded (B=%d T=%d C=%d E=%d I=%d)", B, T, C, E, I);
    EDGL_REQUIRE(c_true >= 0 && c_true <= C, EDGL_ERR_SHAPE, "edgl_dx_encode_bwd_label: true width %d exceeds C=%d", c_true, C);
    EDGL_REQUIRE(lda >= 4 * C && ldb >= 4 * C && lda % 8 == 0 && ldb % 8 == 0, EDGL_ERR_SHAPE,
                 "edgl_dx_encode_bwd_label: bad leading dimensions lda=%d ldb=%d", lda, ldb);
    EDGL_REQUIRE((((uintptr_t)dqkvt | (uintptr_t)W | (uintptr_t)dx0_out) & 15) == 0 &&
                 (((uintptr_t)lab_rows | (uintptr_t)add1 | (uintptr_t)add2) & 7) == 0, EDGL_ERR_SHAPE,
                 "edgl_dx_encode_bwd_label: operands must be 16-byte (GEMM) / 8-byte (rows) aligned");
    EDGL_REQUIRE(drop_rate == 0.f || rng_state, EDGL_ERR_NULL, "edgl_dx_encode_bwd_label: dropout without rng_state");
    hipStream_t st = (hipStream_t)stream;
    const int chunks = (B + G_BM - 1) / G_BM, nbn = 3;
    float* part_pos = workspace;
    float* part_mk = workspace + (long)ENC_NCHUNK * T * C;
    DxEncP x;
    x.e = EncBwdP{ids, marks, nullptr, B, T, C, E, I, drop_rate, rng_state, stream_id, d_item, part_pos, part_mk, chunks, SROWS, add1, add2,
                  sqrtf((float)(c_true > 0 ? c_true : C)), lab_rows, lab_ids, lab_coef, lab_nvalid, lab_R, 1, d_bias, 0, d_mark_emb};
    x.mapT = T; x.mapB = B;
    x.gemm_blocks = xcd_grid(chunks * T * nbn);
    x.lab_blocks = (lab_R + SROWS - 1) / SROWS;
    x.dx0_out = reinterpret_cast<bf16*>(dx0_out);
    const RedJob own[2] = {{part_pos, d_pos, (long)T * C, chunks, T * C, 0, 1}, {part_mk, E > 1 ? d_mark_emb + C : d_mark_emb, (long)C, chunks * T, C, 0, 1}};
    const int nown = E > 1 ? 2 : 1;
    TnRidePlan tn;
    std::memset(&tn.g, 0, sizeof(tn.g));
    int tn_n = 0, tn_blocks = 0;
    if (g_tn_ride && g_tn_defer && g_tn_n > 0) {
        if (tn_ride_plan(g_tn_q, g_tn_n, tn_cus(), nown, &tn)) {
            tn_n = g_tn_n;
            tn_blocks = xcd_grid(tn.blocks);
        } else {
            std::memset(&tn.g, 0, sizeof(tn.g));
            const int rc = tn_flush(st);
            if (rc) return rc;
        }
    }
    RedBatch rb;
    rb.n = rb.blocks = 0;
    int first = 0;
    const int nred = edgl_reduce_ride_take(nullptr, 0, d_item, d_item + (long)I * C, d_bias, d_bias + (I - 1), &rb, &first, st);
    if (nred < 0) return nred;
    StripP p{(const bf16*)dqkvt, (const bf16*)W, dx0_out, B * T, 3 * C, 4 * C, lda, ldb, 3 * C, EpiP{nullptr, nullptr, 0}};
    const size_t smem = std::max((size_t)2 * G_BM * G_LDK * sizeof(bf16), (size_t)DXE_LDS);
    EDGL_LDS_LIMIT(dx_encode_kernel, smem, "edgl_dx_encode_bwd_label");
    g_tn_n -= tn_n;
    hipLaunchKernelGGL(dx_encode_kernel, dim3((unsigned)(tn_blocks + x.gemm_blocks + x.lab_blocks + nred)), dim3(G_NT), smem, st, p, x, rb, tn.g, tn_blocks);
    EDGL_LAUNCH_CHECK();
    if (nred > 0) {
        for (int i = 0; i < nown; ++i) tn.red[i] = own[i];
        return edgl_reduce_rows_now(tn_n ? tn.red : own, tn_n ? tn.nred : nown, st);
    }
    for (int i = 0; i < nown; ++i) {
        const int rc = edgl_reduce_rows_f64(own[i].part, own[i].P, own[i].N, own[i].ld, own[i].out, st);
        if (rc) return rc;
    }
    for (int i = 0; i < tn_n; ++i) {
        const TnP& q = tn.g.job[i];
        const int rc = tn_reduce(q.partial, tn.splits[i], g_tn_q[i].C, q.Kf, q.N, g_tn_q[i].dbias, 0, st);
        if (rc) return rc;
    }
    return EDGL_OK;
}

#ifdef EDGL_PHASE_TIMING
extern "C" int edgl_debug_phase_cycles_gemm(unsigned long long* out16, int reset) {
    if (hipMemcpyFromSymbol(out16, HIP_SYMBOL(gemm2::g_phase_cycles), 16 * sizeof(unsigned long long)) != hipSuccess) return -1;
    if (reset) {
        unsigned long long z[16] = {0};
        if (hipMemcpyToSymbol(HIP_SYMBOL(gemm2::g_phase_cycles), z, sizeof(z)) != hipSuccess) return -1;
    }
    return 0;
}
#endif
```

### easydgl_amd/csrc/tn_group.h

```cpp
#pragma once
#include <algorithm>
#include <cstdint>
#include "red_batch.h"

namespace gemm2 {

constexpr int T_NT = 256, T_BR = 64, T_LD = 128 + 16;

struct TnP {
    const bf16* X; const bf16* Y; int R, Kf, N, ldx, ldy;
    int rows_per_split;
    float* partial;
    int with_colsum;
    int tiles_n, tiles_k, nblocks;
};

constexpr int TN_MAX_JOBS = 8;
struct TnGroupP { TnP job[TN_MAX_JOBS]; int tiles_n[TN_MAX_JOBS], tiles_k[TN_MAX_JOBS], blk0[TN_MAX_JOBS + 1]; int n; };
struct TnQueued { TnP p; float* C; float* dbias; int accumulate, max_splits; };

static inline int tn_choose_splits_on(int cus, int R, int tiles, double flop, double out_elems, int cap) {
    const int smax = std::max(1, std::min(cap, R / 128));
    int best = 1;
    double best_t = 1e30;
    for (int sp = 1; sp <= smax; ++sp) {
        const long wg = (long)tiles * sp;
        const long rounds = (wg + cus - 1) / cus;
        double t = (double)rounds * (flop / (double)wg / (0.6e15 / cus) + 3e-6);
        if (4 * wg < 7L * cus) t *= 1.25;
        if (sp > 1) t += (double)sp * out_elems * 4.0 / 4e12 + 3e-6;
        if (t < best_t * 0.999) { best_t = t; best = sp; }
    }
    return best;
}

static inline int tn_group_layout(TnQueued* q, int n, int cus, TnGroupP* g, int* splits) {
    g->n = n;
    int total_tiles = 0;
    for (int i = 0; i < n; ++i) {
        g->tiles_n[i] = (q[i].p.N + 127) / 128;
        g->tiles_k[i] = (q[i].p.Kf + 127) / 128;
        total_tiles += g->tiles_n[i] * g->tiles_k[i];
    }
    double flop = 0.0, elems = 0.0;
    int rmin = 1 << 30;
    for (int i = 0; i < n; ++i) {
        const TnP& p = q[i].p;
        flop += 2.0 * p.R * p.Kf * p.N;
        elems += (double)(p.Kf + 1) * p.N;
        rmin = std::min(rmin, p.R);
    }
    const int group_splits = tn_choose_splits_on(cus, rmin, total_tiles, flop, elems, 1 << 20);
    int blocks = 0;
    for (int i = 0; i < n; ++i) {
        TnP& p = q[i].p;
        int sp = std::max(1, std::min(std::min(group_splits, q[i].max_splits), p.R / 128));
        const int rps = ((p.R + sp - 1) / sp + T_BR - 1) / T_BR * T_BR;
        sp = (p.R + rps - 1) / rps;
        p.rows_per_split = rps;
        splits[i] = sp;
        g->job[i] = p;
        g->blk0[i] = blocks;
        blocks += g->tiles_n[i] * g->tiles_k[i] * sp;
    }
    g->blk0[n] = blocks;
    return blocks;
}

struct TnRidePlan { TnGroupP g; int blocks, splits[TN_MAX_JOBS]; RedJob red[RED_MAX_JOBS]; int nred; };
static inline int tn_ride_plan(TnQueued* q, int n, int cus, int nown, TnRidePlan* out) {
    if (n <= 0 || n > TN_MAX_JOBS) return 0;
    int nred = nown;
    for (int i = 0; i < n; ++i) {
        const TnP& p = q[i].p;
        if (q[i].accumulate) return 0;
        const bool one = !q[i].dbias || q[i].dbias == q[i].C + (long)p.Kf * p.N;
        if ((((uintptr_t)p.partial | (uintptr_t)q[i].C | (uintptr_t)q[i].dbias) & 15) || (p.N & 3)) return 0;
        nred += one ? 1 : 2;
    }
    if (nred > RED_MAX_JOBS) return 0;
    out->blocks = tn_group_layout(q, n, cus, &out->g, out->splits);
    int k = nown;
    for (int i = 0; i < n; ++i) {
        const TnP& p = q[i].p;
        const long slab = (long)(p.Kf + 1) * p.N;
        const bool with_db = q[i].dbias && q[i].dbias == q[i].C + (long)p.Kf * p.N;
        out->red[k++] = RedJob{p.partial, q[i].C, slab, out->splits[i], (with_db ? p.Kf + 1 : p.Kf) * p.N, 0, 0};
        if (q[i].dbias && !with_db) out->red[k++] = RedJob{p.partial + (long)p.Kf * p.N, q[i].dbias, slab, out->splits[i], p.N, 0, 0};
    }
    out->nred = k;
    return 1;
}

}
```

### easydgl_amd/engine.py

```python
from __future__ import annotations

import ctypes
import os
from typing import Dict, Optional

import torch

from . import _lib, ops
from ._lib import check, lib
from .ops import _ptr, _stream

EPI_BIAS, EPI_GELU, EPI_SAVE_PRE, EPI_MUL_DGELU, EPI_ACCUM, EPI_OUT_F32 = 1, 2, 4, 8, 16, 32


class TrainEngine:
    _SIDE_STREAMS = {}

    def __init__(self, model, batch: int, use_graph: bool = True, process_group=None, fused_tail=None, flash_ce=None,
                 deterministic=None):
        if int(getattr(model, "train_negatives", 0) or 0) > 0:
            raise _lib.EdglError("TrainEngine: the static engine scores the whole catalogue; a model with train_negatives > 0 "
                                 "(sampled-softmax training, DESIGN 4.13) trains on the autograd path: model.train_step")
        if int(getattr(model, "shared_negatives", 0) or 0) > 0:
            raise _lib.EdglError("TrainEngine: the static engine scores the whole catalogue; a model with shared_negatives > 0 "
                                 "(sampled-softmax training, DESIGN 4.15) trains on the autograd path: model.train_step")
        if not getattr(model, "static_engine_ok", True):
            raise _lib.EdglError(f"TrainEngine: {type(model).__name__} is not run by the static engine (DESIGN 4.17: its step, with the "
                                 "model's own Adam hyper-parameters and gradient clipping, is model.train_step / graphed_train_step)")
        env = os.environ.get
        self.sw_flash_ce = env("EDGL_FLASH_CE", "1") != "0"
        self.sw_tpp_fused = env("EDGL_TPP_FUSED", "1") != "0"
        self.sw_prep_in_encoder = env("EDGL_PREP_IN_ENCODER", "1") != "0"
        self.sw_bimau_order = env("EDGL_BIMAU_ORDER", "0") == "1"
        self.sw_ce_parts = env("EDGL_CE_PARTS", "1") != "0"
        self.sw_defer_loss = env("EDGL_DEFER_LOSS", "1") != "0"
        self.sw_adam_ex = env("EDGL_ADAM_EX", "1") != "0"
        self.sw_reduce_ride = env("EDGL_REDUCE_RIDE", "1") != "0"
        self.sw_reduce_ride_behind = env("EDGL_REDUCE_RIDE", "1") == "2"
        self.sw_dx_encode = env("EDGL_DX_ENCODE", "1") != "0"
        self.sw_dw_ride = env("EDGL_DW_RIDE", "1") != "0"
        self.sw_score_strip = env("EDGL_SCORE_STRIP", "1") != "0"
        self.m = model
        self.B = batch
        self.use_graph = use_graph
        self.deterministic = bool(getattr(model, "deterministic", False)) if deterministic is None else bool(deterministic)
        self.group = process_group
        self.graph: Optional[torch.cuda.CUDAGraph] = None
        self.loader = None
        self._feed = False
        self._graph_feeds = False
        m = model
        dev = m._arena.device
        self.dev = dev
        self.dt = m.act_dtype
        self.code = ops._DT[self.dt]
        B, T, C, H, E, M, I = batch, m.seqslen, m.num_units, m.num_heads, m.num_events, m.masklen, m.num_items
        self.T, self.C, self.H, self.E, self.M, self.I = T, C, H, E, M, I
        self.pad = tuple(m.pad)
        self.c_true = int(m.width_true) if self.pad[0] else 0
        self.qk_scale = float(m.qk_scale)
        gmax = int(lib.edgl_bimau_mark_group(C, H, self.code))
        if gmax <= 0:
            raise _lib.EdglError(f"TrainEngine: head dim {C // H} / {self.dt} unsupported by the attention kernels")
        self.mgroups = [(e0, min(E, e0 + gmax)) for e0 in range(0, E, gmax)] if E > gmax else []
        self.R = B * M
        self.rows = B * T
        nb = len(m.layers)
        self.flash_ce = self.sw_flash_ce if flash_ce is None else bool(flash_ce)
        self.fused_tpp = (self.code == _lib.BF16 and C // H == 16 and E == 16 and not self.mgroups and M <= 256 and T <= 128
                          and m.ct_reg != 0.0 and self.flash_ce and nb > 0 and self.sw_tpp_fused)
        e = lambda *s, dtype=None: torch.empty(s, device=dev, dtype=dtype or self.dt)
        f32 = torch.float32
        self.ids = torch.zeros((B, T), device=dev, dtype=torch.int64)
        self.ts = torch.zeros((B, T), device=dev, dtype=f32)
        self.mpos = torch.zeros((B, M), device=dev, dtype=torch.int64)
        self.labels = torch.zeros((B, M), device=dev, dtype=torch.int64)
        self.x0 = e(B, T, 3 * C)
        self.spans = e(B, T, dtype=f32)
        self.marks = e(B, T, E, dtype=torch.uint8)
        self.blk = []
        for i in range(nb):
            d = dict(qkvt=e(B, T, 4 * C), att=e(B, T, C), lam=e(H * B, T, E, dtype=f32), ao=e(B, T, C), a1=e(B, T, C),
                     st1=e(B, 2, dtype=f32), pre_f=e(B, T, 2 * C), f=e(B, T, 2 * C), o=e(B, T, C), y=e(B, T, C),
                     st2=e(B, 2, dtype=f32),
                     pack=e(0 if self.mgroups else lib.edgl_bimau_pack_bytes(C, H, E, self.code), dtype=torch.uint8),
                     saved=e(0 if self.mgroups else lib.edgl_bimau_saved_bytes(B, T, C, H, self.code), dtype=torch.uint8),
                     dlam=None if self.fused_tpp else e(H * B, T, E, dtype=f32),
                     tpp_part=torch.zeros((B * H + 1, 2), device=dev, dtype=f32) if self.fused_tpp else None,
                     tpp=torch.zeros(max(lib.edgl_tpp_workspace(), lib.edgl_tpp_rows_workspace(B, H, M)), device=dev, dtype=f32))
            nb_bits = int(lib.edgl_bimau_dropbits_bytes(B, T, H)) if m.attention_probs_dropout_rate > 0 else 0
            d["dbits"] = e(nb_bits // 4, dtype=torch.int32) if nb_bits > 0 else None
            if self.mgroups:
                dh = C // H
                d["grp"] = []
                for (e0, e1) in self.mgroups:
                    eg = e1 - e0
                    d["grp"].append(dict(
                        marks=e(B, T, eg, dtype=torch.uint8), W1=e(dh + 1, dh * eg, dtype=f32), dW1=e(dh + 1, dh * eg, dtype=f32),
                        pack=e(lib.edgl_bimau_pack_bytes(C, H, eg, self.code), dtype=torch.uint8),
                        saved=e(lib.edgl_bimau_saved_bytes(B, T, C, H, self.code), dtype=torch.uint8),
                        lam=e(H * B, T, eg, dtype=f32), dlam=e(H * B, T, eg, dtype=f32),
                        out=e(B, T, C) if e0 else None, dqkvt=e(B, T, 4 * C) if e0 else None))
            self.blk.append(d)
        self.job_order = (torch.arange(2 * B, device=dev, dtype=torch.int32)
                          if (not self.mgroups and B <= 16384 and nb > 0 and self.sw_bimau_order) else None)
        self.tpp_desc = torch.zeros(int(lib.edgl_tpp_prep_bytes(B, T, M)), device=dev, dtype=torch.uint8) if self.fused_tpp else None
        self.zero_resid = torch.zeros((B, T, C), device=dev, dtype=self.dt) if self.mgroups else None
        self.pre_t, self.so, self.st3 = e(B, T, C), e(B, T, C), e(B, 2, dtype=f32)
        if m.ct_reg != 0.0 and (M > 256 or T > 1024):
            raise _lib.EdglError(f"TrainEngine: masklen {M} > 256 or T {T} > 1024 exceeds the fused TPP kernel (edgl_tpp_fwd_bwd_ex)")
        ok = bool(lib.edgl_tail_supported(T, C, self.code)) and M <= 256
        self.fused_tail = ok if fused_tail is None else (bool(fused_tail) and ok)
        self.tail_pack = [e(int(lib.edgl_tail_pack_elems(C))) for _ in range(nb)] if self.fused_tail else []
        if self.fused_tail:
            self.d_pre_t, self.d_o, self.d_pre_f, self.d_ao = e(B, T, C), e(B, T, C), e(B, T, 2 * C), e(B, T, C)
        self.ws_flash = e(int(lib.edgl_score_flash_workspace(self.R, C, I, I, self.code)), dtype=f32) if self.flash_ce else None
        self.hrows, self.hrows_c = e(self.R, C), e(self.R, C)
        self.hrows_c.zero_()
        self.labels_c = torch.zeros(self.R, device=dev, dtype=torch.int64)
        self.perm, self.inv = e(self.R, dtype=torch.int32), e(self.R, dtype=torch.int32)
        self.nvalid = torch.zeros(1, device=dev, dtype=torch.int32)
        self.lse, self.lab_logit, self.coef = e(self.R, dtype=f32), e(self.R, dtype=f32), e(self.R, dtype=f32)
        self.loss = e(1, dtype=f32)
        self.ce_nparts = int(lib.edgl_score_ce_nparts(self.R, C)) if (self.flash_ce and self.sw_ce_parts) else 0
        self.ce_part = torch.zeros(self.ce_nparts + 1, device=dev, dtype=f32) if self.ce_nparts > 0 else None
        self.loss_aux, self.loss_tpp = torch.zeros(1, device=dev, dtype=f32), torch.zeros(1, device=dev, dtype=f32)
        self.ws_l2 = e(1024, dtype=f32)
        self.l2_nparts = int(lib.edgl_adam_l2_parts(m._arena.numel()))
        self.l2_parts = [torch.zeros(self.l2_nparts, device=dev, dtype=f32) for _ in range(2)] \
            if (m.l2_reg != 0.0 and not use_graph and not self.deterministic) else None
        self._l2p_cur, self._l2p_ready = 0, False
        key = (dev.type, dev.index if dev.index is not None else torch.cuda.current_device())
        if key not in TrainEngine._SIDE_STREAMS:
            TrainEngine._SIDE_STREAMS[key] = (torch.cuda.Stream(device=dev), torch.cuda.Stream(device=dev))
        self.side, self.side2 = TrainEngine._SIDE_STREAMS[key]
        self._pending_loss = None
        self.accumulate_loss = False
        self.loss_sum = torch.zeros(1, device=dev, dtype=torch.float64)
        self._pending_label = None
        self._lazy_loss, self._side_has_grads, self._loss_unjoined = False, False, False
        self._label_fused = False
        self.mau_flags = _lib.MAU_NO_SKIP
        self.adam_ex = (not use_graph) and self.sw_adam_ex and not self.deterministic
        self.reduce_ride = self.sw_reduce_ride and not self.deterministic
        self.dw_ride = self.sw_dw_ride and not self.deterministic
        self._rng_alt, self._adam_alt = torch.zeros_like(m._rng_state), torch.zeros_like(m._adam_state)
        self._slabs = None
        self._slab_info = None
        if self.adam_ex and self.flash_ce:
            info = (ctypes.c_long * 4)()
            check(lib.edgl_score_flash_slab_info(self.R, C, I, I, self.code, info), "edgl_score_flash_slab_info")
            self._slab_info = (int(info[0]), int(info[1]), int(info[2]))
        self._ar_events = None
        self.sync_loss = True
        self._deferred_loss = None
        self._alt = None
        if self.ce_part is not None:
            self._alt = dict(ce_part=torch.zeros_like(self.ce_part), loss_aux=torch.zeros_like(self.loss_aux),
                             tpp_desc=torch.zeros_like(self.tpp_desc) if self.tpp_desc is not None else None,
                             tpp_part=[torch.zeros_like(b["tpp_part"]) if b["tpp_part"] is not None else None for b in self.blk])
        self.counts = torch.zeros(2, device=dev, dtype=torch.int32)
        self._dp = False
        self.d_rows = e(self.R, C)
        self.plan_emb = ops.segsum_plan_buffer(self.rows, I, dev) if self.deterministic else None
        self.plan_lab = ops.segsum_plan_buffer(self.R, I, dev) if self.deterministic else None
        self.G1, self.G2, self.G3, self.G4 = e(B, T, C), e(B, T, C), e(B, T, C), e(B, T, C)
        self.G2c, self.G4c, self.G3c = e(B, T, 2 * C), e(B, T, 4 * C), e(B, T, 3 * C)
        wsz = [2 * self.R * lib.edgl_score_chunks(self.R, I),
               lib.edgl_score_bwd_workspace(self.R, C, I, I, self.code),
               lib.edgl_encode_bwd_workspace(B, T, C), B * 2 * C, 1024]
        for (kf, n) in ((3 * C, 4 * C), (C, 4 * C), (C, C), (C, 2 * C), (2 * C, C)):
            wsz.append(lib.edgl_gemm_dw_workspace(self.rows, kf, n, self.code))
        self.ws = e(max(wsz), dtype=f32)
        self._ws_list, self._ws_i = [], 0
        segs = []
        params = dict(m.named_parameters())
        for n in m.l2_param_names():
            segs += [m._offsets[n], m._offsets[n] + params[n].numel()]
        self.l2_seg = torch.tensor(segs, device=dev, dtype=torch.int64)
        self.nseg = len(segs) // 2

    def _gemm(self, A, Bm, Cm, M, N, K, lda, ldb, ldc, b_kc, bias=None, aux=None, flags=0):
        check(lib.edgl_gemm(_ptr(A), _ptr(Bm), _ptr(Cm), M, N, K, lda, ldb, ldc, 1, int(b_kc), _ptr(bias), _ptr(aux), flags,
                            1, None, self.code, _stream()), "edgl_gemm")

    def _dense_fwd(self, x, dense_kernel, dense_bias, out, K, N, gelu=False, pre=None):
        flags = EPI_BIAS | ((EPI_GELU | EPI_SAVE_PRE) if gelu else 0)
        self._gemm(x, self.m.compute(dense_kernel), out, self.rows, N, K, K, N, N, False, bias=dense_bias, aux=pre, flags=flags)

    def _dense_dx(self, dz, kernel, out, K_in, N, flags=0, aux=None):
        self._gemm(dz, self.m.compute(kernel), out, self.rows, K_in, N, N, N, K_in, True, aux=aux, flags=flags)

    def _ws(self, n, dtype=torch.float32):
        i = self._ws_i
        self._ws_i += 1
        if i == len(self._ws_list):
            self._ws_list.append(torch.empty(max(int(n), 1), device=self.m._arena.device, dtype=dtype))
        w = self._ws_list[i]
        if w.numel() < n or w.dtype != dtype:
            raise _lib.EdglError("TrainEngine: backward launch sequence changed between steps")
        return w

    def _dense_dw(self, x, dz, kernel, bias, K_in, N):
        ws = self._ws(lib.edgl_gemm_dw_workspace(self.rows, K_in, N, self.code))
        check(lib.edgl_gemm_dw(_ptr(x), _ptr(dz), _ptr(kernel.grad), _ptr(bias.grad), self.rows, K_in, N, K_in, N, 0,
                               _ptr(ws), self.code, _stream()), "edgl_gemm_dw")

    def _ln_fwd(self, x, resid, ld_res, ln, drop, y, stats, gpos=None):
        B, T, C = self.B, self.T, self.C
        check(lib.edgl_add_layernorm_fwd_ct(_ptr(x), None if resid is None else resid.data_ptr(), ld_res, _ptr(ln.gamma),
                                            _ptr(ln.beta), B, T, C, float(drop.rate), drop.ptr(), drop.stream_id,
                                            _ptr(gpos), 0 if gpos is None else gpos.shape[1], _ptr(y), _ptr(stats),
                                            self.pad[0], self.pad[1], self.code, _stream()), "edgl_add_layernorm_fwd")

    def _ln_bwd(self, x, resid, ld_res, ln, stats, dy, drop, dsum, dx_drop, gpos=None, rowmap=None, act_pre=None):
        B, T, C = self.B, self.T, self.C
        check(lib.edgl_add_layernorm_bwd_act_ct(_ptr(x), None if resid is None else resid.data_ptr(), ld_res, _ptr(ln.gamma),
                                                _ptr(stats), _ptr(dy), B, T, C, float(drop.rate), drop.ptr(), drop.stream_id,
                                                _ptr(gpos), 0 if gpos is None else gpos.shape[1], _ptr(rowmap), _ptr(act_pre),
                                                _ptr(dsum), _ptr(dx_drop), _ptr(ln.gamma.grad), _ptr(ln.beta.grad),
                                                _ptr(self._ws(B * 2 * C)), self.pad[0], self.pad[1], self.code, _stream()),
              "edgl_add_layernorm_bwd_act")

    def _issue(self, lazy_loss: bool = False, fold_slabs: bool = False):
        m, st = self.m, _stream()
        self._lazy_loss = bool(lazy_loss) and bool(self.blk)
        self._fold = bool(fold_slabs) and self._slab_info is not None and bool(self.blk) and not self._dp
        self._slabs = None
        if self._feed:
            self.loader.write_into(self.ids, self.ts, self.mpos, self.labels)
        if not self._fold:
            m._table_grad_zero = None
        drop = lambda rate, sid: ops.Drop(rate, m._rng_state, sid) if rate > 0 else ops.NO_DROP
        tab = m.item_embs.lookup_table
        tab_c = m.compute(tab)
        l2_from_parts = self.l2_parts is not None and self._l2p_ready and m._state_ahead and m._l2_parts_owner == id(self)
        if not m._state_ahead:
            self._advance_state(st)
        m._state_ahead = False
        main = torch.cuda.current_stream()
        ev_pack = self._issue_side_chain(main, l2_from_parts)
        self._issue_forward(main, ev_pack, drop, tab_c, st)
        lab = self.labels_c
        self._issue_scoring_fwd(tab_c, lab, st)
        self._ws_i = 0
        check(lib.edgl_reduce_defer(1, st), "edgl_reduce_defer")
        try:
            self._issue_backward(st, drop, tab, tab_c, lab)
        except BaseException:
            lib.edgl_reduce_defer(-1, st)
            lib.edgl_gemm_dw_defer(-1, st)
            self._pending_loss = None
            self._pending_label = None
            raise
        check(lib.edgl_reduce_defer(0, st), "edgl_reduce_defer")
        if self._pending_loss is not None:
            self._pending_loss(st)
            self._pending_loss = None
            if self.accumulate_loss:
                self.loss_sum.add_(self.loss)
        if self._lazy_loss and not self._side_has_grads:
            self._loss_unjoined = True
        else:
            torch.cuda.current_stream().wait_stream(self.side)
            self._loss_unjoined = False

    def _l2_term(self, from_parts, sst):
        m = self.m
        if m.l2_reg != 0.0 and from_parts:
            check(lib.edgl_l2_from_parts(_ptr(self.l2_parts[self._l2p_cur]), self.l2_nparts, float(m.l2_reg), _ptr(self.loss_aux), 0,
                                         sst), "edgl_l2_from_parts")
        elif m.l2_reg != 0.0:
            check(lib.edgl_l2_loss(_ptr(m._arena), _ptr(self.l2_seg), self.nseg, float(m.l2_reg), _ptr(self.loss_aux), 0,
                                   _ptr(self.ws_l2), sst), "edgl_l2_loss")

    def _issue_side_chain(self, main, l2_from_parts):
        m = self.m
        B, T, C, H, E, M, R = self.B, self.T, self.C, self.H, self.E, self.M, self.R
        code, ad = self.code, m.attention_probs_dropout_rate
        side, side2 = self.side, self.side2
        sst = side.cuda_stream
        if self._loss_unjoined and self.ce_part is None:
            main.wait_stream(side)
            self._loss_unjoined = False
        side.wait_stream(main)
        if self._deferred_loss is not None:
            a = self._alt
            self.ce_part, a["ce_part"] = a["ce_part"], self.ce_part
            self.loss_aux, a["loss_aux"] = a["loss_aux"], self.loss_aux
            self.tpp_desc, a["tpp_desc"] = a["tpp_desc"], self.tpp_desc
            for j, bj in enumerate(self.blk):
                bj["tpp_part"], a["tpp_part"][j] = a["tpp_part"][j], bj["tpp_part"]
        if not self.sw_prep_in_encoder:
            side2.wait_stream(main)
            if self._loss_unjoined:
                side2.wait_stream(side)
            with torch.cuda.stream(side2):
                check(lib.edgl_compact_scan_labels(_ptr(self.labels), R, _ptr(self.perm), _ptr(self.inv), _ptr(self.nvalid),
# ... 76 lines not shown
                                             _ptr(b["pack"]), B, T, C, H, E, float(da.rate), da.ptr(), da.stream_id, _ptr(b["dbits"]),
                                             self.qk_scale, _ptr(b["att"]), _ptr(b["lam"]), _ptr(b["saved"]),
                                             _ptr(b["dlam"]) if (m.ct_reg != 0.0 and not self.fused_tpp) else None, _ptr(self.job_order),
                                             self.mau_flags, code, st), "edgl_bimau_fwd_ord")
            if m.ct_reg != 0.0 and not self.fused_tpp:
                check(lib.edgl_tpp_fwd_bwd_rows(_ptr(b["lam"]), _ptr(self.mpos), _ptr(self.labels), _ptr(self.ts),
                                                _ptr(m.mark_lookup_table), B, T, H, E, M, float(m.ct_reg / H), _ptr(b["tpp"]),
                                                _ptr(self.loss_tpp), 1 if i > 0 else 0, _ptr(b["dlam"]), st), "edgl_tpp_fwd_bwd_rows")
            if self.fused_tail:
                last = i == len(self.blk) - 1
                pk = self.tail_pack[i]
                dh1 = drop(hd, 11 + 4 * i)
                check(lib.edgl_tail_fwd_ct(_ptr(b["att"]), x.data_ptr(), cin, _ptr(pk), _ptr(blk.att_out.bias), _ptr(blk.inter.bias),
                                        _ptr(blk.out.bias), _ptr(m.transform.bias), _ptr(blk.att_ln.gamma), _ptr(blk.att_ln.beta),
                                        _ptr(blk.out_ln.gamma), _ptr(blk.out_ln.beta), _ptr(m.transform_ln.gamma),
                                        _ptr(m.transform_ln.beta), B, T, C, float(dh1.rate), dh1.ptr(), 11 + 4 * i, 12 + 4 * i,
                                        _ptr(self.mpos), M, int(last), _ptr(b["ao"]), _ptr(b["a1"]), _ptr(b["st1"]), _ptr(b["pre_f"]),
                                        _ptr(b["f"]), _ptr(b["o"]), _ptr(b["y"]), _ptr(b["st2"]), _ptr(self.pre_t), _ptr(self.so),
                                        _ptr(self.st3), _ptr(self.hrows_c), _ptr(self.inv), self.pad[0], self.pad[1], code, st), "edgl_tail_fwd")
            else:
                self._dense_fwd(b["att"], blk.att_out.kernel, blk.att_out.bias, b["ao"], C, C)
                self._ln_fwd(b["ao"], x, cin, blk.att_ln, drop(hd, 11 + 4 * i), b["a1"], b["st1"])
                self._dense_fwd(b["a1"], blk.inter.kernel, blk.inter.bias, b["f"], C, 2 * C, gelu=True, pre=b["pre_f"])
                self._dense_fwd(b["f"], blk.out.kernel, blk.out.bias, b["o"], 2 * C, C)
                self._ln_fwd(b["o"], b["a1"], C, blk.out_ln, drop(hd, 12 + 4 * i), b["y"], b["st2"])
            x, cin = b["y"], C
        if not self.blk:
            main.wait_event(ev_pack)
        if not (self.fused_tail and self.blk):
            self._dense_fwd(x, m.transform.kernel, m.transform.bias, self.so, cin, C, gelu=True, pre=self.pre_t)
            self._ln_fwd(self.so, None, 0, m.transform_ln, ops.NO_DROP, self.hrows, self.st3, gpos=self.mpos)
        if not (self.fused_tail and self.blk):
            check(lib.edgl_compact_gather(_ptr(self.hrows), _ptr(self.labels), _ptr(self.perm), R, C, _ptr(self.hrows_c),
                                          _ptr(self.labels_c), code, st), "edgl_compact_gather")

    def _issue_scoring_fwd(self, tab_c, lab, st):
        m = self.m
        C, I, R, code = self.C, self.I, self.R, self.code
        aux = _ptr(self.loss_aux) if m.l2_reg != 0.0 else None
        tpp = _ptr(self.loss_tpp) if (m.ct_reg != 0.0 and self.blk) else None
        if self.flash_ce:
            wtot = self.counts.data_ptr() if self._dp else None
            check(lib.edgl_score_flash_fwd_rows_wp(_ptr(self.hrows_c), _ptr(tab_c), _ptr(m.output_bias), _ptr(lab), R, C, I,
                                                   _ptr(self.nvalid), wtot, None, _ptr(self.lse), _ptr(self.lab_logit), _ptr(self.coef),
                                                   _ptr(self.d_rows), _ptr(self.ce_part), _ptr(self.ws_flash), code, st),
                  "edgl_score_flash_fwd_rows")
            if self.ce_part is not None:
                self._pending_loss = lambda s, cp=self.ce_part: check(lib.edgl_ce_loss_parts(_ptr(cp), self.ce_nparts, _ptr(self.loss), aux,
                                                                                             tpp, wtot, s), "edgl_ce_loss_parts")
            else:
                self._pending_loss = lambda s: check(lib.edgl_ce_loss_fwd_add_w(_ptr(self.lse), _ptr(self.lab_logit), _ptr(lab), R,
                                                                                _ptr(self.loss), None, aux, tpp, wtot, s),
                                                     "edgl_ce_loss_fwd_add")
        else:
            check(lib.edgl_score_lse_fwd(_ptr(self.hrows_c), _ptr(tab_c), _ptr(m.output_bias), _ptr(lab), R, C, I, 0, I,
                                         _ptr(self.nvalid), _ptr(self.lse), _ptr(self.lab_logit), None, _ptr(self.ws), code, st),
                  "edgl_score_lse_fwd")
            check(lib.edgl_ce_loss_fwd_add_w(_ptr(self.lse), _ptr(self.lab_logit), _ptr(lab), R, _ptr(self.loss), _ptr(self.coef),
                                             aux, tpp, self.counts.data_ptr() if self._dp else None, st), "edgl_ce_loss_fwd_add")
            if self.accumulate_loss:
                self.loss_sum.add_(self.loss)

    def join_loss(self) -> None:
        if self._deferred_loss is not None:
            self.side.wait_stream(torch.cuda.current_stream())
            self._deferred_loss(self.side.cuda_stream)
            self._deferred_loss = None
            self._loss_unjoined = True
        if self._loss_unjoined:
            torch.cuda.current_stream().wait_stream(self.side)
            self._loss_unjoined = False

    def _issue_backward(self, st, drop, tab, tab_c, lab):
        m = self.m
        B, T, C, H, E, M, I, R = self.B, self.T, self.C, self.H, self.E, self.M, self.I, self.R
        code = self.code
        hd, ad = m.hidden_dropout_rate, m.attention_probs_dropout_rate
        if self.flash_ce:
            defer = 1 if (self.blk or self.deterministic) else 0
            if self._fold:
                defer |= 4
                o_t, o_b, ns = self._slab_info
                self._slabs = (self.ws_flash.data_ptr() + 4 * o_t, self.ws_flash.data_ptr() + 4 * o_b, ns)
            check(lib.edgl_score_flash_bwd_ex(_ptr(self.hrows_c), _ptr(tab_c), _ptr(m.output_bias), _ptr(lab), _ptr(self.lse),
                                              _ptr(self.coef), None, R, C, I, 0, I, _ptr(self.nvalid), None,
                                              _ptr(tab.grad), _ptr(m.output_bias.grad), _ptr(self.ws_flash), defer, code, st),
                  "edgl_score_flash_bwd")
            self._label_fused = bool((defer & 1) and self.code == _lib.BF16 and C == 128 and lib.edgl_encode_bwd_label_fused(C, code)
                                     and self.sw_score_strip and not self.deterministic)
            if self.deterministic:
                check(lib.edgl_score_flash_label_term_det(_ptr(self.hrows_c), _ptr(lab), _ptr(self.coef), None, R, C, I, 0, I,
                                                          _ptr(self.nvalid), _ptr(tab.grad), _ptr(m.output_bias.grad),
                                                          _ptr(self.plan_lab), code, st), "edgl_score_flash_label_term_det")
            elif (defer & 1) and not self._label_fused:
                self._pending_label = lambda s: check(lib.edgl_score_flash_label_term(
                    _ptr(self.hrows_c), _ptr(lab), _ptr(self.coef), None, R, C, I, 0, I, _ptr(self.nvalid), _ptr(tab.grad),
                    _ptr(m.output_bias.grad), code, s), "edgl_score_flash_label_term")
        else:
            check(lib.edgl_score_ce_bwd(_ptr(self.hrows_c), _ptr(tab_c), _ptr(m.output_bias), _ptr(lab), _ptr(self.lse),
                                        _ptr(self.coef), None, R, C, I, 0, I, _ptr(self.nvalid), _ptr(self.d_rows), _ptr(tab.grad),
                                        _ptr(m.output_bias.grad), _ptr(self.ws), code, st), "edgl_score_ce_bwd")
        y_last, c_last = (self.blk[-1]["y"], C) if self.blk else (self.x0, 3 * C)
        if not (self.fused_tail and self.blk):
            self._ln_bwd(self.so, None, 0, m.transform_ln, self.st3, self.d_rows, ops.NO_DROP, self.G1, None, gpos=self.mpos,
                         rowmap=self.inv, act_pre=self.pre_t)
            self._dense_dw(y_last, self.G1, m.transform.kernel, m.transform.bias, c_last, C)
            self._dense_dx(self.G1, m.transform.kernel, self.G2 if self.blk else self.G3c, c_last, C)
        dY = self.G2 if self.blk else self.G3c
        for i in reversed(range(len(self.blk))):
            blk, b = m.layers[i], self.blk[i]
            x_in, cin = (self.x0, 3 * C) if i == 0 else (self.blk[i - 1]["y"], C)
            dh2, dh1 = drop(hd, 12 + 4 * i), drop(hd, 11 + 4 * i)
            if self.fused_tail:
                check(lib.edgl_gemm_dw_defer(1, st), "edgl_gemm_dw_defer")
                last = i == len(self.blk) - 1
                tl = m.transform_ln
                check(lib.edgl_tail_bwd_ct(x_in.data_ptr(), cin, _ptr(b["ao"]), _ptr(b["a1"]), _ptr(b["pre_f"]), _ptr(b["o"]),
                                        _ptr(self.pre_t), _ptr(self.so), _ptr(b["st1"]), _ptr(b["st2"]), _ptr(self.st3),
                                        _ptr(m.compute(blk.att_out.kernel)), _ptr(m.compute(blk.inter.kernel)),
                                        _ptr(m.compute(blk.out.kernel)), _ptr(m.compute(m.transform.kernel)),
                                        _ptr(blk.att_ln.gamma), _ptr(blk.out_ln.gamma), _ptr(tl.gamma), B, T, C, float(dh1.rate),
                                        dh1.ptr(), 11 + 4 * i, 12 + 4 * i, int(last), _ptr(self.d_rows), _ptr(self.mpos), M,
                                        _ptr(self.inv), None if last else _ptr(dY), _ptr(self.d_pre_t), _ptr(self.d_o),
                                        _ptr(self.d_pre_f), _ptr(self.d_ao), _ptr(self.G1), _ptr(self.G2),
                                        _ptr(blk.att_ln.gamma.grad), _ptr(blk.att_ln.beta.grad), _ptr(blk.out_ln.gamma.grad),
                                        _ptr(blk.out_ln.beta.grad), _ptr(tl.gamma.grad), _ptr(tl.beta.grad),
                                        _ptr(self._ws(lib.edgl_tail_bwd_workspace(B, C))), self.pad[0], self.pad[1], code, st), "edgl_tail_bwd")
                if self._pending_label is not None:
                    self.side.wait_stream(torch.cuda.current_stream())
                    self._pending_label(self.side.cuda_stream)
                    self._pending_label = None
                if last:
                    self._dense_dw(y_last, self.d_pre_t, m.transform.kernel, m.transform.bias, C, C)
                self._dense_dw(b["f"], self.d_o, blk.out.kernel, blk.out.bias, 2 * C, C)
                self._dense_dw(b["a1"], self.d_pre_f, blk.inter.kernel, blk.inter.bias, C, 2 * C)
                self._dense_dw(b["att"], self.d_ao, blk.att_out.kernel, blk.att_out.bias, C, C)
            else:
                self._ln_bwd(b["o"], b["a1"], C, blk.out_ln, b["st2"], dY, dh2, self.G3, self.G4 if dh2.active else None)
                d_o = self.G4 if dh2.active else self.G3
                self._dense_dw(b["f"], d_o, blk.out.kernel, blk.out.bias, 2 * C, C)
                self._dense_dx(d_o, blk.out.kernel, self.G2c, 2 * C, C, flags=EPI_MUL_DGELU, aux=b["pre_f"])
                self._dense_dw(b["a1"], self.G2c, blk.inter.kernel, blk.inter.bias, C, 2 * C)
                self._dense_dx(self.G2c, blk.inter.kernel, self.G3, C, 2 * C, flags=EPI_ACCUM)
                self._ln_bwd(b["ao"], x_in, cin, blk.att_ln, b["st1"], self.G3, dh1, self.G1, self.G4 if dh1.active else None)
                d_ao = self.G4 if dh1.active else self.G1
                self._dense_dw(b["att"], d_ao, blk.att_out.kernel, blk.att_out.bias, C, C)
                self._dense_dx(d_ao, blk.att_out.kernel, self.G2, C, C)
            att = blk.attention
            da = drop(ad, 10 + 4 * i)
            if self.mgroups:
                self._attention_bwd_groups(att, b, da, st)
            else:
                tp = self.fused_tpp
                check(lib.edgl_bimau_bwd_ord(_ptr(b["qkvt"]), _ptr(self.ids), _ptr(self.spans), _ptr(self.marks), _ptr(b["pack"]),
                                             _ptr(self.G2), None if tp else (_ptr(b["dlam"]) if m.ct_reg != 0.0 else None),
                                             _ptr(self.tpp_desc) if tp else None, M, (_ptr(b["tpp"]) if self._dp else None) if tp else None,
                                             float(m.ct_reg / H), _ptr(b["tpp_part"]) if tp else None,
                                             _ptr(b["lam"]), _ptr(b["saved"]), B, T, C, H, E,
                                             float(da.rate), da.ptr(), da.stream_id, _ptr(b["dbits"]), self.qk_scale, _ptr(self.G4c),
                                             _ptr(att.st_kernel.grad), _ptr(att.st_bias.grad), _ptr(att.weight.grad),
                                             _ptr(att.scaling.grad),
                                             _ptr(self._ws(lib.edgl_bimau_bwd_workspace(B, T, C, H, E, code), torch.uint8)),
                                             _ptr(self.job_order), self.mau_flags, code, st), "edgl_bimau_bwd_ord")
            self._dense_dw(x_in, self.G4c, att.dense_kernel, att.dense_bias, cin, 4 * C)
            dx_encode = i == 0 and self._label_fused and self.sw_dx_encode and not self.deterministic and cin == 3 * C and \
                bool(lib.edgl_dx_encode_supported(B, T, C, code))
            dw_ride = dx_encode and self.dw_ride and self.fused_tail and not self.mgroups
            if self.fused_tail and not dw_ride:
                check(lib.edgl_gemm_dw_defer(0, st), "edgl_gemm_dw_defer")
            d_in = self.G3c if i == 0 else self.G3
            if dx_encode:
                self._issue_backward_end()
                if self.reduce_ride:
                    check(lib.edgl_reduce_ride(2 if self.sw_reduce_ride_behind else 1), "edgl_reduce_ride")
                if dw_ride:
                    check(lib.edgl_gemm_dw_ride(1), "edgl_gemm_dw_ride")
                d0 = drop(hd, 1)
                check(lib.edgl_dx_encode_bwd_label(_ptr(self.G4c), _ptr(self.m.compute(att.dense_kernel)), 4 * C, 4 * C, None,
                                                   _ptr(self.ids), _ptr(self.marks), _ptr(self.G1), _ptr(self.G2), B, T, C, E, I,
                                                   float(d0.rate), d0.ptr(), d0.stream_id, _ptr(tab.grad),
                                                   _ptr(m.pcoding.pembs.lookup_table.grad), _ptr(m.mark_embs.lookup_table.grad),
                                                   _ptr(self._ws(lib.edgl_encode_bwd_workspace(B, T, C))), self.c_true,
                                                   _ptr(self.hrows_c), _ptr(lab), _ptr(self.coef), _ptr(self.nvalid), R,
                                                   _ptr(m.output_bias.grad), code, st), "edgl_dx_encode_bwd_label")
                if dw_ride:
                    check(lib.edgl_gemm_dw_defer(0, st), "edgl_gemm_dw_defer")
                return
            self._dense_dx(self.G4c, att.dense_kernel, d_in, cin, 4 * C)
            if i == 0:
                self._issue_backward_end()
            if i > 0:
                check(lib.edgl_add_cols(_ptr(d_in), cin, _ptr(self.G1), _ptr(self.G2), C, self.rows, C, code, st), "edgl_add_cols")
                self.G2.copy_(self.G3)
                dY = self.G2
            else:
                dY = d_in
        d0 = drop(hd, 1)
        add1, add2 = (self.G1, self.G2) if self.blk else (None, None)
        if self.deterministic:
            check(lib.edgl_encode_bwd_add_det(_ptr(self.ids), _ptr(self.marks), _ptr(dY), _ptr(add1), _ptr(add2), B, T, C, E, I,
                                              float(d0.rate), d0.ptr(), d0.stream_id, _ptr(tab.grad), _ptr(m.pcoding.pembs.lookup_table.grad),
                                              _ptr(m.mark_embs.lookup_table.grad), _ptr(self._ws(lib.edgl_encode_bwd_workspace(B, T, C))),
                                              self.c_true, _ptr(self.plan_emb), code, st), "edgl_encode_bwd_add_det")
            return
        if self.reduce_ride:
            check(lib.edgl_reduce_ride(2 if self.sw_reduce_ride_behind else 1), "edgl_reduce_ride")
        if self._label_fused:
            check(lib.edgl_encode_bwd_add_label(_ptr(self.ids), _ptr(self.marks), _ptr(dY), _ptr(add1), _ptr(add2), B, T, C, E, I,
                                                float(d0.rate), d0.ptr(), d0.stream_id, _ptr(tab.grad),
                                                _ptr(m.pcoding.pembs.lookup_table.grad), _ptr(m.mark_embs.lookup_table.grad),
                                                _ptr(self._ws(lib.edgl_encode_bwd_workspace(B, T, C))), self.c_true,
                                                _ptr(self.hrows_c), _ptr(lab), _ptr(self.coef), _ptr(self.nvalid), R,
                                                _ptr(m.output_bias.grad), code, st), "edgl_encode_bwd_add_label")
        else:
            check(lib.edgl_encode_bwd_add_ct(_ptr(self.ids), _ptr(self.marks), _ptr(dY), _ptr(add1), _ptr(add2), B, T, C, E, I,
                                             float(d0.rate), d0.ptr(), d0.stream_id, _ptr(tab.grad), _ptr(m.pcoding.pembs.lookup_table.grad),
                                             _ptr(m.mark_embs.lookup_table.grad), _ptr(self._ws(lib.edgl_encode_bwd_workspace(B, T, C))),
                                             self.c_true, code, st), "edgl_encode_bwd_add")

    def _issue_backward_end(self):
        m = self.m
        B, H = self.B, self.H
        pending, self._pending_loss = self._pending_loss, None

        def loss_launches(s, pending=pending, parts=[bj["tpp_part"] for bj in self.blk]):
            if self.fused_tpp:
                for j, bj in enumerate(self.blk):
                    check(lib.edgl_tpp_finish_parts_n(_ptr(parts[j]), B * H, float(m.ct_reg / H), H, _ptr(bj["tpp"]),
                                                      _ptr(self.loss_tpp), 1 if j > 0 else 0, s), "edgl_tpp_finish_parts")
            if pending is not None:
                pending(s)
                if self.accumulate_loss:
                    with torch.cuda.stream(self.side):
                        self.loss_sum.add_(self.loss)

        self._side_has_grads = self._pending_label is not None
        if self._lazy_loss and not self.sync_loss and not self._side_has_grads and self.ce_part is not None and \
                (self.fused_tpp or m.ct_reg == 0.0) and self.sw_defer_loss:
            self._deferred_loss = loss_launches
        else:
            self.side.wait_stream(torch.cuda.current_stream())
            loss_launches(self.side.cuda_stream)
        if self._pending_label is not None:
            self._pending_label(self.side.cuda_stream)
            self._pending_label = None
        if not self._lazy_loss or self._side_has_grads:
            check(lib.edgl_reduce_flush(self.side.cuda_stream), "edgl_reduce_flush")

    def _attention_fwd_groups(self, b, x, cin, da, st):
        m = self.m
        B, T, C, H, E, code = self.B, self.T, self.C, self.H, self.E, self.code
        for g, ((e0, e1), gb) in enumerate(zip(self.mgroups, b["grp"])):
            gb["marks"].copy_(self.marks[:, :, e0:e1])
            first = g == 0
            check(lib.edgl_bimau_fwd_db(_ptr(b["qkvt"]), x.data_ptr() if first else self.zero_resid.data_ptr(), cin if first else C,
                                        _ptr(self.ids), _ptr(self.spans), _ptr(gb["marks"]), _ptr(gb["pack"]), B, T, C, H, e1 - e0,
                                        float(da.rate), da.ptr(), da.stream_id, _ptr(b["dbits"]), self.qk_scale, _ptr(b["att"] if first else gb["out"]),
                                        _ptr(gb["lam"]), _ptr(gb["saved"]), None, 0 if first else ops.MAU_DIAG_ZERO, code, st),
                  "edgl_bimau_fwd_db")
            if not first:
                check(lib.edgl_add(_ptr(b["att"]), _ptr(gb["out"]), _ptr(b["att"]), b["att"].numel(), code, st), "edgl_add")
        torch.cat([gb["lam"] for gb in b["grp"]], dim=-1, out=b["lam"])
        if m.ct_reg != 0.0:
            b["dlam"].zero_()

    def _attention_bwd_groups(self, att, b, da, st):
        m = self.m
        B, T, C, H, code = self.B, self.T, self.C, self.H, self.code
        dh = C // H
        check(lib.edgl_reduce_defer(0, st), "edgl_reduce_defer")
        for g, ((e0, e1), gb) in enumerate(zip(self.mgroups, b["grp"])):
            first = g == 0
            if m.ct_reg != 0.0:
                gb["dlam"].copy_(b["dlam"][:, :, e0:e1])
            check(lib.edgl_bimau_bwd_db(_ptr(b["qkvt"]), _ptr(self.ids), _ptr(self.spans), _ptr(gb["marks"]), _ptr(gb["pack"]),
                                     _ptr(self.G2), _ptr(gb["dlam"]) if m.ct_reg != 0.0 else None, _ptr(gb["lam"]), _ptr(gb["saved"]),
                                     B, T, C, H, e1 - e0, float(da.rate), da.ptr(), da.stream_id, _ptr(b["dbits"]), self.qk_scale,
                                     _ptr(self.G4c if first else gb["dqkvt"]), _ptr(gb["dW1"]), _ptr(att.st_bias.grad[e0 * dh:e1 * dh]),
                                     _ptr(att.weight.grad[e0:e1]), _ptr(att.scaling.grad[e0:e1]),
                                     _ptr(self._ws(lib.edgl_bimau_bwd_workspace(B, T, C, H, e1 - e0, code), torch.uint8)),
                                     0 if first else ops.MAU_DIAG_ZERO, code, st), "edgl_bimau_bwd")
            att.st_kernel.grad[:, e0 * dh:e1 * dh].copy_(gb["dW1"])
            if not first:
                check(lib.edgl_add(_ptr(self.G4c), _ptr(gb["dqkvt"]), _ptr(self.G4c), self.G4c.numel(), code, st), "edgl_add")
        check(lib.edgl_reduce_defer(1, st), "edgl_reduce_defer")

    def _advance_state(self, st):
        m = self.m
        check(lib.edgl_step_begin(_ptr(m._rng_state), _ptr(m._adam_state), float(m.learning_rate), 0.9, 0.999, st),
              "edgl_step_begin")

    def _optimizer(self):
        m = self.m
        m.mask_padded_grads()
        seg = self.l2_seg if m.l2_reg != 0.0 else None
        if self.adam_ex and not m._state_pinned:
            l2p = None
            if self.l2_parts is not None and seg is not None:
                self._l2p_cur ^= 1
                l2p = self.l2_parts[self._l2p_cur]
            tab, ob = m.item_embs.lookup_table, m.output_bias
            a0 = m._arena.data_ptr()
            sl = self._slabs
            self._slabs = None
            lo_a, lo_b = (tab.data_ptr() - a0) // 4, (ob.data_ptr() - a0) // 4
            check(lib.edgl_adam_apply_ex(_ptr(m._arena), _ptr(m._grad_arena), _ptr(m._adam_m), _ptr(m._adam_v), m._arena.numel(), 0.9, 0.999,
                                         1e-8, _ptr(m._adam_state), float(m.l2_reg), _ptr(seg), 0 if seg is None else seg.numel() // 2,
                                         _ptr(m._shadow), _ptr(l2p),
                                         ctypes.c_void_p(sl[0]) if sl else None, tab.numel(), lo_a, lo_a + tab.numel(), self.C,
                                         ctypes.c_void_p(sl[1]) if sl else None, ob.numel(), lo_b, lo_b + ob.numel(), sl[2] if sl else 0,
                                         _ptr(m._rng_state), _ptr(self._adam_alt), _ptr(self._rng_alt), float(m.learning_rate), _stream()),
                  "edgl_adam_apply_ex")
            if l2p is not None:
                self._l2p_ready = True
                m._l2_parts_owner = id(self)
            else:
                m._l2_parts_owner = None
            m._table_grad_zero = id(self) if sl else None
            m._rng_state, self._rng_alt = self._rng_alt, m._rng_state
            m._adam_state, self._adam_alt = self._adam_alt, m._adam_state
            m._state_ahead = True
            return
        if self._slabs is not None:
            raise _lib.EdglError("TrainEngine: the scoring gradient's slabs were left for edgl_adam_apply_ex, which is not in use")
        if self.l2_parts is not None and seg is not None:
            self._l2p_cur ^= 1
            check(lib.edgl_adam_apply_l2p(_ptr(m._arena), _ptr(m._grad_arena), _ptr(m._adam_m), _ptr(m._adam_v), m._arena.numel(), 0.9,
                                          0.999, 1e-8, _ptr(m._adam_state), float(m.l2_reg), _ptr(seg), seg.numel() // 2, _ptr(m._shadow),
# ... 152 lines not shown
```

Measured before the change: 737,800.

## Run deferred weight-gradient TN GEMM tiles as riders inside bimau backward sweep 1

Queued deferred dW TN GEMM products are now executed as extra workgroups prepended to the bimau backward sweep-1 launch, instead of running in a separate grouped launch or riding in dx_encode. The goal is to fill idle CUs during the attention backward sweep and drop one launch and its tail. The split reductions for those products are deferred (the 'gone' list) and handled later by the dx_encode reduce or at flush. The TN body moves into a shared header. Risks: launch_bounds(256,3) on the rider variant may limit registers for the attention sweep, and the rider tiles compete with it for CUs.

```diff
diff --git a/easydgl_amd/build.py b/easydgl_amd/build.py
--- a/easydgl_amd/build.py
+++ b/easydgl_amd/build.py
@@ -11,7 +11,7 @@
 OUT = os.path.join(HERE, "libeasydgl_hip.so")
 SOURCES = ["k_misc.hip", "k_tpp.hip", "k_optim.hip", "k_adam_rows.hip", "k_reduce.hip", "k_data.hip", "k_encode.hip", "k_gemm.hip", "k_gemm2.hip", "k_layernorm.hip", "k_bimau_fwd.hip", "k_bimau_bwd.hip", "k_bimau_big.hip", "k_bimau_stream.hip",
            "k_score.hip", "k_ce.hip", "k_score_strip.hip", "k_score_stripw.hip", "k_eval_tile.hip", "k_eval_topk.hip", "k_eval_rank.hip", "k_eval_cand.hip", "k_cand_ce.hip", "k_shared_ce.hip", "k_sampled_loss.hip", "k_tattn.hip", "k_tiattn.hip", "k_timefn.hip", "k_coding.hip", "k_tail.hip", "k_segsum.hip", "k_gru.hip", "k_s2pnm.hip", "k_mate.hip", "k_tahe.hip"]
-HEADERS = ["edgl_common.h", "lds_limit.h", "batch_prep.h", "tpp_math.h", "score_plan.h", "topk_select.h", "gemm_tile.h", "bimau_common.h", "bimau_fwd_impl.h", "bimau_bwd_impl.h", "red_batch.h", "tn_group.h", "encode_scatter.h", "strip_mma.h", "score_strip.h", "eval_sweep.h", "cand_gather.h", "sampled_dv.h", "tattn_common.h", os.path.join("..", "..", "include", "easydgl_hip.h")]
+HEADERS = ["edgl_common.h", "lds_limit.h", "batch_prep.h", "tpp_math.h", "score_plan.h", "topk_select.h", "gemm_tile.h", "bimau_common.h", "bimau_fwd_impl.h", "bimau_bwd_impl.h", "red_batch.h", "tn_group.h", "tn_body.h", "encode_scatter.h", "strip_mma.h", "score_strip.h", "eval_sweep.h", "cand_gather.h", "sampled_dv.h", "tattn_common.h", os.path.join("..", "..", "include", "easydgl_hip.h")]
 FLAGS = ["--offload-arch=gfx950", "-O3", "-std=c++17", "-fPIC", "-munsafe-fp-atomics", "-Wno-unused-result"]
 EXTRA_FLAGS = {"k_bimau_fwd.hip": ["-mllvm", "-amdgpu-mfma-vgpr-form=1"],
                "k_bimau_bwd.hip": ["-mllvm", "-amdgpu-mfma-vgpr-form=1"],
diff --git a/easydgl_amd/csrc/bimau_bwd_impl.h b/easydgl_amd/csrc/bimau_bwd_impl.h
--- a/easydgl_amd/csrc/bimau_bwd_impl.h
+++ b/easydgl_amd/csrc/bimau_bwd_impl.h
@@ -2,6 +2,7 @@
 #include <algorithm>
 
 #include "bimau_common.h"
+#include "tn_body.h"
 
 #ifdef EDGL_PHASE_TIMING
 extern __device__ unsigned long long g_phase_cycles[16];
@@ -63,13 +64,27 @@
     else *reinterpret_cast<uint2*>(dst) = *reinterpret_cast<uint2*>(&f);
 }
 
-template <typename T, int DT, int NT, int EC, bool PREF = true, int FL = -1, bool DB = false, bool TP = false, bool SK = false>
-__global__ __launch_bounds__(256) void bimau_bwd_sweep1_kernel(BwdP p) {
+template <bool RIDE> struct SweepRide {};
+template <> struct SweepRide<true> { gemm2::TnGroupP g; int blocks; };
+template <typename T, int DT, int NT, int EC, bool PREF = true, int FL = -1, bool DB = false, bool TP = false, bool SK = false, bool RIDE = false>
+__global__ __launch_bounds__(256, RIDE ? 3 : 1) void bimau_bwd_sweep1_kernel(BwdP p, SweepRide<RIDE> rd) {
+    static_assert(sizeof(BwdP) + sizeof(SweepRide<true>) < 4096, "kernel arguments: 4 KB");
     constexpr int dh = 16 * DT, Tp = 16 * NT, LDT = Tp + 4;
     extern __shared__ __attribute__((aligned(16))) char smem[];
+    int bid = (int)blockIdx.x;
+    if constexpr (RIDE) {
+        static_assert(sizeof(T) == 2 && DT == 1 && FL == 0 && EC == 16 && NT <= 7, "riders: the headline family");
+        static_assert(gemm2::T_NT == 256, "the TN tiles run in this kernel's workgroup shape");
+        if (bid < rd.blocks) {
+            const int vid = gemm2::xcd_virtual_id(bid, rd.blocks, rd.g.blk0[rd.g.n]);
+            if (vid >= 0) gemm2::tn_group_tile(rd.g, vid, reinterpret_cast<bf16*>(smem));
+            return;
+        }
+        bid -= rd.blocks;
+    }
     const int E = EC ? EC : p.E;
     const int lane = threadIdx.x & 63, wave = __builtin_amdgcn_readfirstlane(threadIdx.x >> 6);
-    const long slot = (long)blockIdx.x * p.waves + wave;
+    const long slot = (long)bid * p.waves + wave;
     if (slot >= (long)p.B * p.H) return;
     const int sb = (int)(slot / p.H), head = (int)(slot % p.H);
     const int b = p.order ? __builtin_amdgcn_readfirstlane(p.order[sb]) : sb;
diff --git a/easydgl_amd/csrc/k_bimau_big.hip b/easydgl_amd/csrc/k_bimau_big.hip
--- a/easydgl_amd/csrc/k_bimau_big.hip
+++ b/easydgl_amd/csrc/k_bimau_big.hip
@@ -482,7 +482,7 @@
         p.waves = waves;
         auto kern = bimau_bwd_sweep1_kernel<T, DT, NT, 0, false>;
         EDGL_LDS_LIMIT(kern, smem, "edgl_bimau_bwd");
-        hipLaunchKernelGGL(kern, dim3((unsigned)((jobs + waves - 1) / waves)), dim3(64 * waves), smem, st, p);
+        hipLaunchKernelGGL(kern, dim3((unsigned)((jobs + waves - 1) / waves)), dim3(64 * waves), smem, st, p, SweepRide<false>{});
         EDGL_LAUNCH_CHECK();
     }
     {
diff --git a/easydgl_amd/csrc/k_bimau_bwd.hip b/easydgl_amd/csrc/k_bimau_bwd.hip
--- a/easydgl_amd/csrc/k_bimau_bwd.hip
+++ b/easydgl_amd/csrc/k_bimau_bwd.hip
@@ -370,9 +370,29 @@
                 }
             }
         }
-        EDGL_LDS_LIMIT(kern, smem, "edgl_bimau_bwd");
-        hipLaunchKernelGGL(kern, dim3((unsigned)((jobs + waves - 1) / waves)), dim3(64 * waves), smem, st, p);
-        EDGL_LAUNCH_CHECK();
+        bool rode = false;
+        if constexpr (SPEC && NT <= 7) {
+            if (p.flags == 0 && p.E == 16 && waves * 64 == gemm2::T_NT && !(bimau_skip_enabled() && !p.noskip)) {
+                SweepRide<true> rd;
+                rd.blocks = edgl_gemm2_tn_sweep_take(p.B * p.T, 3 * p.C, 4 * p.C, &rd.g);
+                if (rd.blocks > 0) {
+                    const bool db = p.dbits && p.rate > 0.f;
+                    auto kr = bimau_bwd_sweep1_kernel<T, DT, NT, 16, true, 0, false, false, false, true>;
+                    if (p.tpp_desc) kr = db ? bimau_bwd_sweep1_kernel<T, DT, NT, 16, true, 0, true, true, false, true> : bimau_bwd_sweep1_kernel<T, DT, NT, 16, true, 0, false, true, false, true>;
+                    else if (db) kr = bimau_bwd_sweep1_kernel<T, DT, NT, 16, true, 0, true, false, false, true>;
+                    const size_t smem_r = std::max(smem, (size_t)2 * gemm2::T_BR * gemm2::T_LD * sizeof(bf16));
+                    EDGL_LDS_LIMIT(kr, smem_r, "edgl_bimau_bwd (riders)");
+                    hipLaunchKernelGGL(kr, dim3((unsigned)((jobs + waves - 1) / waves + rd.blocks)), dim3(64 * waves), smem_r, st, p, rd);
+                    EDGL_LAUNCH_CHECK();
+                    rode = true;
+                }
+            }
+        }
+        if (!rode) {
+            EDGL_LDS_LIMIT(kern, smem, "edgl_bimau_bwd");
+            hipLaunchKernelGGL(kern, dim3((unsigned)((jobs + waves - 1) / waves)), dim3(64 * waves), smem, st, p, SweepRide<false>{});
+            EDGL_LAUNCH_CHECK();
+        }
     }
     {
         const int rc = launch_intensity_bwd<T, DT>(p, jobs, st);
diff --git a/easydgl_amd/csrc/k_gemm2.hip b/easydgl_amd/csrc/k_gemm2.hip
--- a/easydgl_amd/csrc/k_gemm2.hip
+++ b/easydgl_amd/csrc/k_gemm2.hip
@@ -3,35 +3,14 @@
 #include "edgl_common.h"
 #include <cstring>
 #include "encode_scatter.h"
-#include "tn_group.h"
-
-typedef __attribute__((ext_vector_type(4))) short tr_s16x4;
+#include "tn_body.h"
 
 namespace gemm2 {
-
-__device__ __forceinline__ uint2 tr_read(const bf16* tile, int ld, int k0, int z0, int lane) {
-    const int G = lane >> 4, s = lane & 15;
-    const bf16* p = tile + (k0 + 4 * G + (s >> 2)) * ld + z0 + 4 * (s & 3);
-    tr_s16x4 v = __builtin_amdgcn_ds_read_tr16_b64_v4i16((__attribute__((address_space(3))) tr_s16x4*)p);
-    return *reinterpret_cast<uint2*>(&v);
-}
-__device__ __forceinline__ bf16x8 tr_frag32(const bf16* tile, int ld, int k0, int z0, int lane) {
-    bf16x8 f;
-    *reinterpret_cast<uint2*>(&f) = tr_read(tile, ld, k0, z0, lane);
-    *(reinterpret_cast<uint2*>(&f) + 1) = tr_read(tile, ld, k0 + 16, z0, lane);
-    return f;
-}
 
 struct EpiP {
     const float* bias; void* aux; int flags;
 };
 
-__device__ __forceinline__ int xcd_virtual_id(int b, int grid, int n_real) {
-    if (grid & 7) return b < n_real ? b : -1;
-    const int v = (b & 7) * (grid >> 3) + (b >> 3);
-    return v < n_real ? v : -1;
-}
-static inline int xcd_grid(int n_real) { return (n_real + 7) / 8 * 8; }
 __device__ __forceinline__ void epi_store4(const EpiP& e, bf16* C, void* Cany, long idx, int n, float x[4]) {
     if (e.flags & EDGL_EPI_BIAS) {
         const float4 b = *reinterpret_cast<const float4*>(e.bias + n);
@@ -632,9 +611,6 @@
     }
 }
 
-template <int TM>
-__device__ __forceinline__ void tn_body(const TnP& p, int bx, int by, int bz, bf16* Xs, bf16* Ys);
-
 __global__ __launch_bounds__(G_NT, 3) void dx_encode_kernel(StripP p, DxEncP x, RedBatch rb, TnGroupP g, int tn_blocks) {
     static_assert(sizeof(StripP) + sizeof(DxEncP) + sizeof(RedBatch) + sizeof(TnGroupP) + sizeof(int) < 4096, "kernel arguments: 4 KB");
     static_assert(T_NT == G_NT && 2 * T_BR * T_LD * (int)sizeof(bf16) <= DXE_LDS, "the TN tiles run in this kernel's workgroup shape and LDS");
@@ -681,101 +657,6 @@
 }
 
 template <int TM>
-__device__ __forceinline__ void tn_body(const TnP& p, int bx, int by, int bz, bf16* Xs, bf16* Ys) {
-    constexpr int NI = TM / 32, LDT = TM + 16, PCS = TM / 8, NLD = T_BR * PCS / T_NT;
-    const int tid = threadIdx.x, lane = tid & 63, wave = tid >> 6, wm = wave >> 1, wn = wave & 1;
-    const int g4 = (lane >> 4) * 4, l15 = lane & 15;
-    const int kf0 = by * TM, n0 = bx * TM;
-    const int r_lo = bz * p.rows_per_split, r_hi = min(p.R, r_lo + p.rows_per_split);
-    f32x4 acc[NI][NI];
-#pragma unroll
-    for (int i = 0; i < NI; ++i)
-#pragma unroll
-        for (int j = 0; j < NI; ++j) acc[i][j] = f32x4{0.f, 0.f, 0.f, 0.f};
-    constexpr int NCS = NI / 2;
-    f32x4 acc_cs[NCS];
-#pragma unroll
-    for (int j = 0; j < NCS; ++j) acc_cs[j] = f32x4{0.f, 0.f, 0.f, 0.f};
-    const bool do_cs = p.with_colsum && by == 0;
-    bf16x8 ones;
-#pragma unroll
-    for (int i = 0; i < 8; ++i) ones[i] = (__bf16)1.0f;
-    uint4 px[NLD], py[NLD];
-    int r0_cur = 0;
-    auto load = [&](int r0) {
-        r0_cur = r0;
-#pragma unroll
-        for (int i = 0; i < NLD; ++i) {
-            const int v = tid + i * T_NT, row = v / PCS, cv = v % PCS, gr = min(r0 + row, r_hi - 1);
-            const int cx = min(kf0 + cv * 8, p.Kf - 8), cy = min(n0 + cv * 8, p.N - 8);
-            px[i] = *reinterpret_cast<const uint4*>(p.X + (long)gr * p.ldx + cx);
-            py[i] = *reinterpret_cast<const uint4*>(p.Y + (long)gr * p.ldy + cy);
-        }
-    };
-    auto store = [&]() {
-#pragma unroll
-        for (int i = 0; i < NLD; ++i) {
-            const int v = tid + i * T_NT, row = v / PCS, cv = v % PCS;
-            const bool ok = r0_cur + row < r_hi;
-            *reinterpret_cast<uint4*>(Xs + row * LDT + cv * 8) = ok ? px[i] : make_uint4(0, 0, 0, 0);
-            *reinterpret_cast<uint4*>(Ys + row * LDT + cv * 8) = ok ? py[i] : make_uint4(0, 0, 0, 0);
-        }
-    };
-    const int nstep = (r_hi - r_lo + T_BR - 1) / T_BR;
-    if (nstep > 0) { load(r_lo); store(); }
-    __syncthreads();
-    for (int st = 0; st < nstep; ++st) {
-        const bool more = st + 1 < nstep;
-        if (more) load(r_lo + (st + 1) * T_BR);
-#pragma unroll
-        for (int rb = 0; rb < T_BR / 32; ++rb) {
-            bf16x8 af[NI], bf_[NI];
-#pragma unroll
-            for (int i = 0; i < NI; ++i) af[i] = tr_frag32(Xs, LDT, rb * 32, wm * (TM / 2) + i * 16, lane);
-#pragma unroll
-            for (int j = 0; j < NI; ++j) bf_[j] = tr_frag32(Ys, LDT, rb * 32, wn * (TM / 2) + j * 16, lane);
-#pragma unroll
-            for (int i = 0; i < NI; ++i)
-#pragma unroll
-                for (int j = 0; j < NI; ++j) acc[i][j] = __builtin_amdgcn_mfma_f32_16x16x32_bf16(af[i], bf_[j], acc[i][j], 0, 0, 0);
-            if (do_cs) {
-                if (wm) {
-#pragma unroll
-                    for (int j = 0; j < NCS; ++j) acc_cs[j] = __builtin_amdgcn_mfma_f32_16x16x32_bf16(ones, bf_[NCS + j], acc_cs[j], 0, 0, 0);
-                } else {
-#pragma unroll
-                    for (int j = 0; j < NCS; ++j) acc_cs[j] = __builtin_amdgcn_mfma_f32_16x16x32_bf16(ones, bf_[j], acc_cs[j], 0, 0, 0);
-                }
-            }
-        }
-        lds_barrier();
-        if (more) store();
-        lds_barrier();
-    }
-    float* out = p.partial + (long)bz * (p.Kf + 1) * p.N;
-#pragma unroll
-    for (int i = 0; i < NI; ++i)
-#pragma unroll
-        for (int r = 0; r < 4; ++r) {
-            const int kf = kf0 + wm * (TM / 2) + i * 16 + g4 + r;
-            if (kf < p.Kf) {
-#pragma unroll
-                for (int j = 0; j < NI; ++j) {
-                    const int n = n0 + wn * (TM / 2) + j * 16 + l15;
-                    if (n < p.N) out[(long)kf * p.N + n] = acc[i][j][r];
-                }
-            }
-        }
-    if (do_cs && lane < 16) {
-#pragma unroll
-        for (int j = 0; j < NCS; ++j) {
-            const int n = n0 + wn * (TM / 2) + (wm * NCS + j) * 16 + lane;
-            if (n < p.N) out[(long)p.Kf * p.N + n] = acc_cs[j][0];
-        }
-    }
-}
-
-template <int TM>
 __global__ __launch_bounds__(T_NT) void tn_gemm_kernel(TnP p) {
     extern __shared__ __attribute__((aligned(16))) char tn_smem[];
     bf16* Xs = reinterpret_cast<bf16*>(tn_smem);
@@ -898,15 +779,30 @@
 thread_local bool g_tn_defer = false;
 thread_local int g_tn_n = 0;
 thread_local TnQueued g_tn_q[TN_MAX_JOBS];
-thread_local bool g_tn_ride = false;
+thread_local int g_tn_ride = 0;
+thread_local TnGone g_tn_gone = {{}, {}, 0};
+
+static int tn_gone_reduce(hipStream_t st) {
+    const int n = g_tn_gone.n;
+    g_tn_gone.n = 0;
+    for (int i = 0; i < n; ++i) {
+        const TnQueued& e = g_tn_gone.q[i];
+        const int rc = tn_reduce(e.p.partial, g_tn_gone.splits[i], e.C, e.p.Kf, e.p.N, e.dbias, e.accumulate, st);
+        if (rc) return rc;
+    }
+    return EDGL_OK;
+}
 
 static int tn_flush(hipStream_t st) {
     const int n = g_tn_n;
     g_tn_n = 0;
+    const TnAlso also = tn_gone_also(&g_tn_gone);
+    const int rc0 = tn_gone_reduce(st);
+    if (rc0) return rc0;
     if (n == 0) return EDGL_OK;
     TnGroupP g;
     int splits[TN_MAX_JOBS];
-    const int blocks = tn_group_layout(g_tn_q, n, tn_cus(), &g, splits);
+    const int blocks = tn_group_layout(g_tn_q, n, tn_cus(), &g, splits, &also);
     const size_t tn_lds = (size_t)2 * T_BR * (128 + 16) * sizeof(bf16);
     EDGL_LDS_LIMIT(tn_gemm_group_kernel, tn_lds, "edgl_gemm_dw (grouped)");
     hipLaunchKernelGGL(tn_gemm_group_kernel, dim3(xcd_grid(blocks)), dim3(T_NT), tn_lds, st, g);
@@ -920,8 +816,8 @@
 }
 
 int edgl_gemm2_tn_defer(int on, hipStream_t st) {
-    if (on <= 0) g_tn_ride = false;
-    if (on < 0) { g_tn_n = 0; g_tn_defer = false; return EDGL_OK; }
+    if (on <= 0) g_tn_ride = 0;
+    if (on < 0) { g_tn_n = 0; g_tn_gone.n = 0; g_tn_defer = false; return EDGL_OK; }
     if (!on && g_tn_defer) {
         g_tn_defer = false;
         return tn_flush(st);
@@ -957,9 +853,19 @@
 }
 
 extern "C" int edgl_gemm_dw_ride(int on) {
-    EDGL_REQUIRE(on == 0 || on == 1, EDGL_ERR_SHAPE, "edgl_gemm_dw_ride: on = %d (0: off, 1: the queued products ride in the launch of edgl_dx_encode_bwd_label)", on);
-    g_tn_ride = on != 0;
+    EDGL_REQUIRE(on >= 0 && on <= 2, EDGL_ERR_SHAPE, "edgl_gemm_dw_ride: on = %d (0: off, 1: the queued products ride in the launch of "
+                 "edgl_dx_encode_bwd_label, 2: in sweep 1 of the next edgl_bimau_bwd call)", on);
+    g_tn_ride = on;
     return EDGL_OK;
+}
+
+int edgl_gemm2_tn_sweep_take(int R2, int Kf2, int N2, gemm2::TnGroupP* g) {
+    if (g_tn_ride != 2) return 0;
+    g_tn_ride = 1;
+    if (!g_tn_defer || g_tn_n == 0 || g_tn_gone.n != 0) return 0;
+    if (!tn_sweep_plan(g_tn_q, g_tn_n, tn_cus(), R2, Kf2, N2, g, &g_tn_gone)) return 0;
+    g_tn_n = 0;
+    return xcd_grid(g->blk0[g->n]);
 }
 
 extern "C" int edgl_dx_encode_supported(int B, int T, int C, int dtype) {
@@ -1003,9 +909,11 @@
     TnRidePlan tn;
     std::memset(&tn.g, 0, sizeof(tn.g));
     int tn_n = 0, tn_blocks = 0;
-    if (g_tn_ride && g_tn_defer && g_tn_n > 0) {
-        if (tn_ride_plan(g_tn_q, g_tn_n, tn_cus(), nown, &tn)) {
+    int gone_n = 0;
+    if (g_tn_ride && g_tn_defer && (g_tn_n > 0 || g_tn_gone.n > 0)) {
+        if (tn_ride_plan(g_tn_q, g_tn_n, tn_cus(), nown, &tn, &g_tn_gone)) {
             tn_n = g_tn_n;
+            gone_n = g_tn_gone.n;
             tn_blocks = xcd_grid(tn.blocks);
         } else {
             std::memset(&tn.g, 0, sizeof(tn.g));
@@ -1026,10 +934,15 @@
     EDGL_LAUNCH_CHECK();
     if (nred > 0) {
         for (int i = 0; i < nown; ++i) tn.red[i] = own[i];
+        if (tn_n) g_tn_gone.n = 0;
         return edgl_reduce_rows_now(tn_n ? tn.red : own, tn_n ? tn.nred : nown, st);
     }
     for (int i = 0; i < nown; ++i) {
         const int rc = edgl_reduce_rows_f64(own[i].part, own[i].P, own[i].N, own[i].ld, own[i].out, st);
+        if (rc) return rc;
+    }
+    if (gone_n) {
+        const int rc = tn_gone_reduce(st);
         if (rc) return rc;
     }
     for (int i = 0; i < tn_n; ++i) {
diff --git a/easydgl_amd/csrc/tn_body.h b/easydgl_amd/csrc/tn_body.h
--- /dev/null
+++ b/easydgl_amd/csrc/tn_body.h
@@ -0,0 +1,135 @@
+#pragma once
+#include "edgl_common.h"
+#include "tn_group.h"
+
+typedef __attribute__((ext_vector_type(4))) short tr_s16x4;
+
+namespace gemm2 {
+
+__device__ __forceinline__ uint2 tr_read(const bf16* tile, int ld, int k0, int z0, int lane) {
+    const int G = lane >> 4, s = lane & 15;
+    const bf16* p = tile + (k0 + 4 * G + (s >> 2)) * ld + z0 + 4 * (s & 3);
+    tr_s16x4 v = __builtin_amdgcn_ds_read_tr16_b64_v4i16((__attribute__((address_space(3))) tr_s16x4*)p);
+    return *reinterpret_cast<uint2*>(&v);
+}
+__device__ __forceinline__ bf16x8 tr_frag32(const bf16* tile, int ld, int k0, int z0, int lane) {
+    bf16x8 f;
+    *reinterpret_cast<uint2*>(&f) = tr_read(tile, ld, k0, z0, lane);
+    *(reinterpret_cast<uint2*>(&f) + 1) = tr_read(tile, ld, k0 + 16, z0, lane);
+    return f;
+}
+
+__device__ __forceinline__ int xcd_virtual_id(int b, int grid, int n_real) {
+    if (grid & 7) return b < n_real ? b : -1;
+    const int v = (b & 7) * (grid >> 3) + (b >> 3);
+    return v < n_real ? v : -1;
+}
+static inline int xcd_grid(int n_real) { return (n_real + 7) / 8 * 8; }
+
+template <int TM>
+__device__ __forceinline__ void tn_body(const TnP& p, int bx, int by, int bz, bf16* Xs, bf16* Ys) {
+    constexpr int NI = TM / 32, LDT = TM + 16, PCS = TM / 8, NLD = T_BR * PCS / T_NT;
+    const int tid = threadIdx.x, lane = tid & 63, wave = tid >> 6, wm = wave >> 1, wn = wave & 1;
+    const int g4 = (lane >> 4) * 4, l15 = lane & 15;
+    const int kf0 = by * TM, n0 = bx * TM;
+    const int r_lo = bz * p.rows_per_split, r_hi = min(p.R, r_lo + p.rows_per_split);
+    f32x4 acc[NI][NI];
+#pragma unroll
+    for (int i = 0; i < NI; ++i)
+#pragma unroll
+        for (int j = 0; j < NI; ++j) acc[i][j] = f32x4{0.f, 0.f, 0.f, 0.f};
+    constexpr int NCS = NI / 2;
+    f32x4 acc_cs[NCS];
+#pragma unroll
+    for (int j = 0; j < NCS; ++j) acc_cs[j] = f32x4{0.f, 0.f, 0.f, 0.f};
+    const bool do_cs = p.with_colsum && by == 0;
+    bf16x8 ones;
+#pragma unroll
+    for (int i = 0; i < 8; ++i) ones[i] = (__bf16)1.0f;
+    uint4 px[NLD], py[NLD];
+    int r0_cur = 0;
+    auto load = [&](int r0) {
+        r0_cur = r0;
+#pragma unroll
+        for (int i = 0; i < NLD; ++i) {
+            const int v = tid + i * T_NT, row = v / PCS, cv = v % PCS, gr = min(r0 + row, r_hi - 1);
+            const int cx = min(kf0 + cv * 8, p.Kf - 8), cy = min(n0 + cv * 8, p.N - 8);
+            px[i] = *reinterpret_cast<const uint4*>(p.X + (long)gr * p.ldx + cx);
+            py[i] = *reinterpret_cast<const uint4*>(p.Y + (long)gr * p.ldy + cy);
+        }
+    };
+    auto store = [&]() {
+#pragma unroll
+        for (int i = 0; i < NLD; ++i) {
+            const int v = tid + i * T_NT, row = v / PCS, cv = v % PCS;
+            const bool ok = r0_cur + row < r_hi;
+            *reinterpret_cast<uint4*>(Xs + row * LDT + cv * 8) = ok ? px[i] : make_uint4(0, 0, 0, 0);
+            *reinterpret_cast<uint4*>(Ys + row * LDT + cv * 8) = ok ? py[i] : make_uint4(0, 0, 0, 0);
+        }
+    };
+    const int nstep = (r_hi - r_lo + T_BR - 1) / T_BR;
+    if (nstep > 0) { load(r_lo); store(); }
+    __syncthreads();
+    for (int st = 0; st < nstep; ++st) {
+        const bool more = st + 1 < nstep;
+        if (more) load(r_lo + (st + 1) * T_BR);
+#pragma unroll
+        for (int rb = 0; rb < T_BR / 32; ++rb) {
+            bf16x8 af[NI], bf_[NI];
+#pragma unroll
+            for (int i = 0; i < NI; ++i) af[i] = tr_frag32(Xs, LDT, rb * 32, wm * (TM / 2) + i * 16, lane);
+#pragma unroll
+            for (int j = 0; j < NI; ++j) bf_[j] = tr_frag32(Ys, LDT, rb * 32, wn * (TM / 2) + j * 16, lane);
+#pragma unroll
+            for (int i = 0; i < NI; ++i)
+#pragma unroll
+                for (int j = 0; j < NI; ++j) acc[i][j] = __builtin_amdgcn_mfma_f32_16x16x32_bf16(af[i], bf_[j], acc[i][j], 0, 0, 0);
+            if (do_cs) {
+                if (wm) {
+#pragma unroll
+                    for (int j = 0; j < NCS; ++j) acc_cs[j] = __builtin_amdgcn_mfma_f32_16x16x32_bf16(ones, bf_[NCS + j], acc_cs[j], 0, 0, 0);
+                } else {
+#pragma unroll
+                    for (int j = 0; j < NCS; ++j) acc_cs[j] = __builtin_amdgcn_mfma_f32_16x16x32_bf16(ones, bf_[j], acc_cs[j], 0, 0, 0);
+                }
+            }
+        }
+        lds_barrier();
+        if (more) store();
+        lds_barrier();
+    }
+    float* out = p.partial + (long)bz * (p.Kf + 1) * p.N;
+#pragma unroll
+    for (int i = 0; i < NI; ++i)
+#pragma unroll
+        for (int r = 0; r < 4; ++r) {
+            const int kf = kf0 + wm * (TM / 2) + i * 16 + g4 + r;
+            if (kf < p.Kf) {
+#pragma unroll
+                for (int j = 0; j < NI; ++j) {
+                    const int n = n0 + wn * (TM / 2) + j * 16 + l15;
+                    if (n < p.N) out[(long)kf * p.N + n] = acc[i][j][r];
+                }
+            }
+        }
+    if (do_cs && lane < 16) {
+#pragma unroll
+        for (int j = 0; j < NCS; ++j) {
+            const int n = n0 + wn * (TM / 2) + (wm * NCS + j) * 16 + lane;
+            if (n < p.N) out[(long)p.Kf * p.N + n] = acc_cs[j][0];
+        }
+    }
+}
+
+__device__ __forceinline__ void tn_group_tile(const TnGroupP& g, int vid, bf16* Xs) {
+    int j = 0;
+    for (int i = 1; i < g.n; ++i)
+        if (vid >= g.blk0[i]) j = i;
+    const int local = vid - g.blk0[j];
+    const int tn = g.tiles_n[j], tk = g.tiles_k[j];
+    tn_body<128>(g.job[j], local % tn, (local / tn) % tk, local / (tn * tk), Xs, Xs + T_BR * T_LD);
+}
+
+}
+
+int edgl_gemm2_tn_sweep_take(int R2, int Kf2, int N2, gemm2::TnGroupP* g);
diff --git a/easydgl_amd/csrc/tn_group.h b/easydgl_amd/csrc/tn_group.h
--- a/easydgl_amd/csrc/tn_group.h
+++ b/easydgl_amd/csrc/tn_group.h
@@ -34,23 +34,24 @@
     return best;
 }
 
-static inline int tn_group_layout(TnQueued* q, int n, int cus, TnGroupP* g, int* splits) {
+struct TnAlso { int tiles; double flop, elems; int rmin; };
+static inline TnAlso tn_also_none() { return TnAlso{0, 0.0, 0.0, 1 << 30}; }
+static inline void tn_also_add(TnAlso* a, int R, int Kf, int N) {
+    a->tiles += ((Kf + 127) / 128) * ((N + 127) / 128);
+    a->flop += 2.0 * R * Kf * N;
+    a->elems += (double)(Kf + 1) * N;
+    a->rmin = std::min(a->rmin, R);
+}
+
+static inline int tn_group_layout(TnQueued* q, int n, int cus, TnGroupP* g, int* splits, const TnAlso* also = nullptr) {
     g->n = n;
-    int total_tiles = 0;
+    TnAlso all = also ? *also : tn_also_none();
     for (int i = 0; i < n; ++i) {
         g->tiles_n[i] = (q[i].p.N + 127) / 128;
         g->tiles_k[i] = (q[i].p.Kf + 127) / 128;
-        total_tiles += g->tiles_n[i] * g->tiles_k[i];
+        tn_also_add(&all, q[i].p.R, q[i].p.Kf, q[i].p.N);
     }
-    double flop = 0.0, elems = 0.0;
-    int rmin = 1 << 30;
-    for (int i = 0; i < n; ++i) {
-        const TnP& p = q[i].p;
-        flop += 2.0 * p.R * p.Kf * p.N;
-        elems += (double)(p.Kf + 1) * p.N;
-        rmin = std::min(rmin, p.R);
-    }
-    const int group_splits = tn_choose_splits_on(cus, rmin, total_tiles, flop, elems, 1 << 20);
+    const int group_splits = tn_choose_splits_on(cus, all.rmin, all.tiles, all.flop, all.elems, 1 << 20);
     int blocks = 0;
     for (int i = 0; i < n; ++i) {
         TnP& p = q[i].p;
@@ -67,29 +68,64 @@
     return blocks;
 }
 
+static inline int tn_red_count(const TnQueued& e) {
+    const TnP& p = e.p;
+    if (e.accumulate) return 0;
+    if ((((uintptr_t)p.partial | (uintptr_t)e.C | (uintptr_t)e.dbias) & 15) || (p.N & 3)) return 0;
+    return !e.dbias || e.dbias == e.C + (long)p.Kf * p.N ? 1 : 2;
+}
+static inline int tn_red_jobs(const TnQueued& e, int splits, RedJob* out) {
+    const TnP& p = e.p;
+    const long slab = (long)(p.Kf + 1) * p.N;
+    const bool with_db = e.dbias && e.dbias == e.C + (long)p.Kf * p.N;
+    int k = 0;
+    out[k++] = RedJob{p.partial, e.C, slab, splits, (with_db ? p.Kf + 1 : p.Kf) * p.N, 0, 0};
+    if (e.dbias && !with_db) out[k++] = RedJob{p.partial + (long)p.Kf * p.N, e.dbias, slab, splits, p.N, 0, 0};
+    return k;
+}
+
+struct TnGone { TnQueued q[TN_MAX_JOBS]; int splits[TN_MAX_JOBS]; int n; };
+static inline TnAlso tn_gone_also(const TnGone* gone) {
+    TnAlso a = tn_also_none();
+    for (int i = 0; gone && i < gone->n; ++i) tn_also_add(&a, gone->q[i].p.R, gone->q[i].p.Kf, gone->q[i].p.N);
+    return a;
+}
+
 struct TnRidePlan { TnGroupP g; int blocks, splits[TN_MAX_JOBS]; RedJob red[RED_MAX_JOBS]; int nred; };
-static inline int tn_ride_plan(TnQueued* q, int n, int cus, int nown, TnRidePlan* out) {
+static inline int tn_ride_plan(TnQueued* q, int n, int cus, int nown, TnRidePlan* out, const TnGone* gone = nullptr) {
     if (n <= 0 || n > TN_MAX_JOBS) return 0;
     int nred = nown;
+    for (int i = 0; gone && i < gone->n; ++i) nred += tn_red_count(gone->q[i]);
     for (int i = 0; i < n; ++i) {
-        const TnP& p = q[i].p;
-        if (q[i].accumulate) return 0;
-        const bool one = !q[i].dbias || q[i].dbias == q[i].C + (long)p.Kf * p.N;
-        if ((((uintptr_t)p.partial | (uintptr_t)q[i].C | (uintptr_t)q[i].dbias) & 15) || (p.N & 3)) return 0;
-        nred += one ? 1 : 2;
+        const int c = tn_red_count(q[i]);
+        if (!c) return 0;
+        nred += c;
     }
     if (nred > RED_MAX_JOBS) return 0;
-    out->blocks = tn_group_layout(q, n, cus, &out->g, out->splits);
+    const TnAlso also = tn_gone_also(gone);
+    out->blocks = tn_group_layout(q, n, cus, &out->g, out->splits, &also);
     int k = nown;
-    for (int i = 0; i < n; ++i) {
-        const TnP& p = q[i].p;
-        const long slab = (long)(p.Kf + 1) * p.N;
-        const bool with_db = q[i].dbias && q[i].dbias == q[i].C + (long)p.Kf * p.N;
-        out->red[k++] = RedJob{p.partial, q[i].C, slab, out->splits[i], (with_db ? p.Kf + 1 : p.Kf) * p.N, 0, 0};
-        if (q[i].dbias && !with_db) out->red[k++] = RedJob{p.partial + (long)p.Kf * p.N, q[i].dbias, slab, out->splits[i], p.N, 0, 0};
-    }
+    for (int i = 0; gone && i < gone->n; ++i) k += tn_red_jobs(gone->q[i], gone->splits[i], out->red + k);
+    for (int i = 0; i < n; ++i) k += tn_red_jobs(q[i], out->splits[i], out->red + k);
     out->nred = k;
     return 1;
 }
 
+static inline int tn_sweep_plan(TnQueued* q, int n, int cus, int R2, int Kf2, int N2, TnGroupP* g, TnGone* gone) {
+    if (n <= 0 || n > TN_MAX_JOBS) return 0;
+    int nred = 2 + 2;
+    for (int i = 0; i < n; ++i) {
+        const int c = tn_red_count(q[i]);
+        if (!c) return 0;
+        nred += c;
+    }
+    if (nred > RED_MAX_JOBS) return 0;
+    TnAlso also = tn_also_none();
+    tn_also_add(&also, R2, Kf2, N2);
+    tn_group_layout(q, n, cus, g, gone->splits, &also);
+    for (int i = 0; i < n; ++i) gone->q[i] = q[i];
+    gone->n = n;
+    return 1;
 }
+
+}
diff --git a/easydgl_amd/engine.py b/easydgl_amd/engine.py
--- a/easydgl_amd/engine.py
+++ b/easydgl_amd/engine.py
@@ -39,6 +39,7 @@
         self.sw_reduce_ride_behind = env("EDGL_REDUCE_RIDE", "1") == "2"
         self.sw_dx_encode = env("EDGL_DX_ENCODE", "1") != "0"
         self.sw_dw_ride = env("EDGL_DW_RIDE", "1") != "0"
+        self.sw_dw_ride_sweep = env("EDGL_DW_RIDE_SWEEP", "1") != "0"
         self.sw_score_strip = env("EDGL_SCORE_STRIP", "1") != "0"
         self.m = model
         self.B = batch
@@ -144,6 +145,8 @@
         self.adam_ex = (not use_graph) and self.sw_adam_ex and not self.deterministic
         self.reduce_ride = self.sw_reduce_ride and not self.deterministic
         self.dw_ride = self.sw_dw_ride and not self.deterministic
+        self.dw_ride_sweep = self.dw_ride and self.sw_dw_ride_sweep and not use_graph and self.code == _lib.BF16 and \
+            self.C // self.H == 16 and self.E == 16 and self.T <= 112
         self._rng_alt, self._adam_alt = torch.zeros_like(m._rng_state), torch.zeros_like(m._adam_state)
         self._slabs = None
         self._slab_info = None
@@ -526,6 +529,10 @@
                 self._attention_bwd_groups(att, b, da, st)
             else:
                 tp = self.fused_tpp
+                sweep_ride = i == 0 and self.dw_ride_sweep and self.fused_tail and not self._dp and self._label_fused and \
+                    self.sw_dx_encode and cin == 3 * C and bool(lib.edgl_dx_encode_supported(B, T, C, code))
+                if sweep_ride:
+                    check(lib.edgl_gemm_dw_ride(2), "edgl_gemm_dw_ride")
                 check(lib.edgl_bimau_bwd_ord(_ptr(b["qkvt"]), _ptr(self.ids), _ptr(self.spans), _ptr(self.marks), _ptr(b["pack"]),
                                              _ptr(self.G2), None if tp else (_ptr(b["dlam"]) if m.ct_reg != 0.0 else None),
                                              _ptr(self.tpp_desc) if tp else None, M, (_ptr(b["tpp"]) if self._dp else None) if tp else None,
@@ -547,7 +554,7 @@
                 self._issue_backward_end()
                 if self.reduce_ride:
                     check(lib.edgl_reduce_ride(2 if self.sw_reduce_ride_behind else 1), "edgl_reduce_ride")
-                if dw_ride:
+                if dw_ride and not sweep_ride:
                     check(lib.edgl_gemm_dw_ride(1), "edgl_gemm_dw_ride")
                 d0 = drop(hd, 1)
                 check(lib.edgl_dx_encode_bwd_label(_ptr(self.G4c), _ptr(self.m.compute(att.dense_kernel)), 4 * C, 4 * C, None,
```

Result: no change. 740,800 (median of 6 runs) (+0.4%).
